# nomadoor/ComfyUI-Video-Stabilizer

Measured on AMD Instinct MI355X. Metric: stabilized frames/sec (1080p, similarity mode), higher is better.
Workload: dtype f32; 1 GPU; C2: 256-frame clip, 1920x1080, Video Stabilizer Flow (DIS) similarity + crop_and_pad, defaults (strength 0.7, smooth 0.5, 16 fps), device-resident in/out, entered at the node's input adaptation; frames_per_gpu=256, total_frames=256

## Files before the change

### comfyui-video-stabilizer_amd/csrc/vstab_api.hip

```cpp
#include "vstab_internal.h"
#include <cmath>
#include <cstdarg>

static thread_local char g_err[1024] = "";

void vstab_set_error(const char* fmt, ...)
{
    va_list ap;
    va_start(ap, fmt);
    vsnprintf(g_err, sizeof(g_err), fmt, ap);
    va_end(ap);
}

int ScratchBuf::reserve(size_t need)
{
    if (need <= bytes) return 0;
    size_t want = need + need / 4 + 256;
    if (ptr) {
        if (pinned_host) (void)hipHostFree(ptr);
        else (void)hipFree(ptr);
        ptr = nullptr;
        bytes = 0;
    }
    hipError_t e = pinned_host ? hipHostMalloc(&ptr, want, hipHostMallocDefault) : hipMalloc(&ptr, want);
    if (e != hipSuccess) {
        vstab_set_error("scratch allocation of %zu bytes failed: %s", want, hipGetErrorString(e));
        ptr = nullptr;
        return 1;
    }
    bytes = want;
    return 0;
}

void ScratchBuf::release()
{
    if (ptr) {
        if (pinned_host) (void)hipHostFree(ptr);
        else (void)hipFree(ptr);
    }
    ptr = nullptr;
    bytes = 0;
}

bool vstab_invert3x3(const double* S, double* D) { return vstab_invert3x3_hd(S, D); }

int vstab_stage_params(vstab_ctx* ctx, const void* host, size_t bytes, void** dev_out)
{
    VSTAB_HIP(hipEventSynchronize(ctx->ev_params_free));
    if (ctx->h_params.reserve(bytes)) return 1;
    if (ctx->d_params.reserve(bytes)) return 1;
    memcpy(ctx->h_params.ptr, host, bytes);
    VSTAB_HIP(hipMemcpyAsync(ctx->d_params.ptr, ctx->h_params.ptr, bytes, hipMemcpyHostToDevice, ctx->stream));
    VSTAB_HIP(hipEventRecord(ctx->ev_params_free, ctx->stream));
    *dev_out = ctx->d_params.ptr;
    return 0;
}

EventPair* vstab_timer_slot(vstab_ctx* ctx, const char* kind)
{
    auto it = ctx->timers.find(kind);
    if (it == ctx->timers.end()) {
        EventPair ep;
        if (hipEventCreate(&ep.start) != hipSuccess || hipEventCreate(&ep.stop) != hipSuccess) return nullptr;
        it = ctx->timers.emplace(kind, ep).first;
    }
    return &it->second;
}

int vstab_timer_fold(EventPair* ev)
{
    if (!ev->pending) return 0;
    float ms = 0.f;
    VSTAB_HIP(hipEventSynchronize(ev->stop));
    VSTAB_HIP(hipEventElapsedTime(&ms, ev->start, ev->stop));
    ev->total_ms += ms;
    ev->launches += 1;
    ev->pending = false;
    return 0;
}

int vstab_check_device_status(vstab_ctx* ctx, const char* who)
{
    if (!ctx || !ctx->h_status) return 0;
// ... 9 lines not shown
    return 3;
}

void vstab_tvl1_release(vstab_ctx* ctx);

extern "C" {

int vstab_abi_version(void) { return VSTAB_ABI_VERSION; }

int vstab_test_hooks(void)
{
#ifdef VSTAB_TEST_HOOKS
    return 1;
#else
    return 0;
#endif
}

const char* vstab_last_error(void) { return g_err; }

int vstab_create(vstab_ctx** out, int device)
{
    VSTAB_REQUIRE(out != nullptr, "vstab_create: out is NULL");
    int count = 0;
    VSTAB_HIP(hipGetDeviceCount(&count));
    VSTAB_REQUIRE(count > 0, "vstab_create: no HIP device visible");
    if (device < 0) VSTAB_HIP(hipGetDevice(&device));
    VSTAB_REQUIRE(device < count, "vstab_create: device %d out of range (%d visible)", device, count);
    VSTAB_HIP(hipSetDevice(device));
    vstab_ctx* ctx = new vstab_ctx();
    ctx->device = device;
    ctx->h_params.pinned_host = true;
    ctx->h_fit.pinned_host = true;
    ctx->h_xfer.pinned_host = true;
    VSTAB_HIP(hipEventCreateWithFlags(&ctx->ev_params_free, hipEventDisableTiming));
    VSTAB_HIP(hipEventRecord(ctx->ev_params_free, nullptr));
    {
        void* h = nullptr;
        VSTAB_HIP(hipHostMalloc(&h, 64, hipHostMallocMapped | hipHostMallocCoherent));
        memset(h, 0, 64);
        void* d = nullptr;
        VSTAB_HIP(hipHostGetDevicePointer(&d, h, 0));
        ctx->h_status = static_cast<volatile int*>(h);
        ctx->d_status = static_cast<int*>(d);
    }
    *out = ctx;
    return 0;
}

int vstab_destroy(vstab_ctx* ctx)
{
    if (!ctx) return 0;
    (void)hipSetDevice(ctx->device);
    (void)hipStreamSynchronize(ctx->stream);
    ctx->h_params.release();
    ctx->d_params.release();
    ctx->d_dis.release();
    vstab_tvl1_release(ctx);
    ctx->d_fit.release();
    ctx->h_fit.release();
    ctx->d_gray_tmp.release();
    ctx->d_range.release();
    ctx->d_mask_rows.release();
    ctx->d_plan.release();
    ctx->h_plan.release();
    if (ctx->h_peaks) (void)hipHostFree(ctx->h_peaks);
    if (ctx->d_peaks_count) (void)hipFree(ctx->d_peaks_count);
    if (ctx->h_counts) (void)hipHostFree(ctx->h_counts);
    if (ctx->ev_fit_done) (void)hipEventDestroy(ctx->ev_fit_done);
    if (ctx->ev_plan_done) (void)hipEventDestroy(ctx->ev_plan_done);
    if (ctx->side_stream) { (void)hipStreamSynchronize(ctx->side_stream); (void)hipStreamDestroy(ctx->side_stream); }
    if (ctx->ev_side) (void)hipEventDestroy(ctx->ev_side);
    for (auto& kv : ctx->timers) { (void)hipEventDestroy(kv.second.start); (void)hipEventDestroy(kv.second.stop); }
    (void)hipEventDestroy(ctx->ev_params_free);
    if (ctx->h_status) (void)hipHostFree(const_cast<int*>(ctx->h_status));
    if (ctx->xfer_stream) { (void)hipStreamSynchronize(ctx->xfer_stream); (void)hipStreamDestroy(ctx->xfer_stream); }
    for (auto& ev : ctx->ev_xfer) if (ev) (void)hipEventDestroy(ev);
    if (ctx->ev_xfer_sync) (void)hipEventDestroy(ctx->ev_xfer_sync);
    ctx->h_xfer.release();
    ctx->d_xfer.release();
    if (ctx->prep_stream) { (void)hipStreamSynchronize(ctx->prep_stream); (void)hipStreamDestroy(ctx->prep_stream); }
    for (auto& ev : ctx->ev_prep) if (ev) (void)hipEventDestroy(ev);
    if (ctx->ev_pyramid) (void)hipEventDestroy(ctx->ev_pyramid);
    delete ctx;
    return 0;
}

int vstab_set_stream(vstab_ctx* ctx, void* hip_stream)
{
    VSTAB_REQUIRE(ctx != nullptr, "vstab_set_stream: ctx is NULL");
    ctx->stream = reinterpret_cast<hipStream_t>(hip_stream);
    return 0;
}

int vstab_synchronize(vstab_ctx* ctx)
{
    VSTAB_REQUIRE(ctx != nullptr, "vstab_synchronize: ctx is NULL");
    VSTAB_HIP(hipStreamSynchronize(ctx->stream));
    return vstab_check_device_status(ctx, "vstab_synchronize");
}


int vstab_set_timing(vstab_ctx* ctx, int enabled)
{
    VSTAB_REQUIRE(ctx != nullptr, "vstab_set_timing: ctx is NULL");
    ctx->timing = enabled != 0;
    ctx->timing_detail = enabled == 2;
    ctx->timing_warp_only = enabled == 3;
    for (auto& kv : ctx->timers) { kv.second.pending = false; kv.second.total_ms = 0.0; kv.second.launches = 0; }
    return 0;
}

int vstab_last_kernel_ms(vstab_ctx* ctx, const char* kind, float* ms_out)
{
    VSTAB_REQUIRE(ctx != nullptr && kind != nullptr && ms_out != nullptr, "vstab_last_kernel_ms: NULL argument");
    auto it = ctx->timers.find(kind);
    VSTAB_REQUIRE(it != ctx->timers.end() && it->second.start != nullptr && (it->second.pending || it->second.launches > 0),
                  "vstab_last_kernel_ms: no timing recorded for '%s'", kind);
    VSTAB_HIP(hipEventSynchronize(it->second.stop));
    VSTAB_HIP(hipEventElapsedTime(ms_out, it->second.start, it->second.stop));
    return 0;
}

int vstab_kernel_ms_stats(vstab_ctx* ctx, const char* kind, double* total_ms, int* launches)
{
    VSTAB_REQUIRE(ctx != nullptr && kind != nullptr && total_ms != nullptr && launches != nullptr, "vstab_kernel_ms_stats: NULL argument");
    auto it = ctx->timers.find(kind);
    VSTAB_REQUIRE(it != ctx->timers.end(), "vstab_kernel_ms_stats: no timing recorded for '%s'", kind);
    if (int rc = vstab_timer_fold(&it->second)) return rc;
    *total_ms = it->second.total_ms;
    *launches = it->second.launches;
    return 0;
}

int vstab_host_math(int op, const double* a, const double* b, int n, double* out)
{
    VSTAB_REQUIRE(a != nullptr && out != nullptr && n >= 0, "vstab_host_math: bad argument");
    VSTAB_REQUIRE(op >= VSTAB_HOST_SQRT && op <= VSTAB_HOST_SIN, "vstab_host_math: unknown op %d", op);
    VSTAB_REQUIRE(op != VSTAB_HOST_ATAN2 || b != nullptr, "vstab_host_math: atan2 needs two inputs");
    for (int i = 0; i < n; i++) {
        switch (op) {
        case VSTAB_HOST_SQRT: out[i] = std::sqrt(a[i]); break;
        case VSTAB_HOST_ATAN2: out[i] = std::atan2(a[i], b[i]); break;
        case VSTAB_HOST_LOG: out[i] = std::log(a[i]); break;
        case VSTAB_HOST_EXP: out[i] = std::exp(a[i]); break;
        case VSTAB_HOST_COS: out[i] = std::cos(a[i]); break;
        default: out[i] = std::sin(a[i]); break;
        }
    }
    return 0;
}

int vstab_transitions_to_params(const float* work_mats, int count, int mode, const double* up, const double* down,
                                float* full_mats, double* params)
{
    VSTAB_REQUIRE(count >= 0 && (count == 0 || (work_mats && full_mats && params)), "vstab_transitions_to_params: bad argument");
    VSTAB_REQUIRE(mode >= VSTAB_MODE_TRANSLATION && mode <= VSTAB_MODE_PERSPECTIVE, "vstab_transitions_to_params: unknown mode %d", mode);
    VSTAB_REQUIRE((up == nullptr) == (down == nullptr), "vstab_transitions_to_params: up and down come together");
    for (int n = 0; n < count; n++) {
        const float* M = work_mats + (size_t)n * 9;
        float* F = full_mats + (size_t)n * 9;
        for (int i = 0; i < 3; i++)
            for (int j = 0; j < 3; j++) {
                if (up) {
                    const double t = up[i] * (double)M[i * 3 + j];
                    F[i * 3 + j] = (float)(t * down[j]);
// ... 85 lines not shown
```

### comfyui-video-stabilizer_amd/csrc/vstab_dis.hip

```cpp
#include "vstab_internal.h"
#include <cstdlib>
#include <cfloat>
#include <algorithm>
#include <cmath>
#include <memory>

namespace {

constexpr float DIS_EPS = 0.001f;
constexpr float DIS_INF = 1e10f;
constexpr int DIS_BORDER = 16;
constexpr int PSZ = 8;
constexpr int PSTR = 4;
constexpr int DEFAULT_FINEST = 2;
constexpr int GD_ITERS = 25;
constexpr int VAR_ITERS = 5;
constexpr int SOR_ITERS = 5;
constexpr int MAX_LEVELS = 16;

struct LevelGeom {
    int w, h, ws, hs;
};

unsigned grid_for(long long items, int block = 256)
{
    long long b = (items + block - 1) / block;
    const long long cap = 256LL * 32;
    if (b > cap) b = cap;
    if (b < 1) b = 1;
    return (unsigned)b;
}

dim3 frame_grid(long long per_frame, int frames, int block = 256)
{
    long long b = (per_frame + block - 1) / block;
    const long long cap = std::max(1LL, (256LL * 32) / std::max(frames, 1));
    if (b > cap) b = cap;
    if (b < 1) b = 1;
    return dim3((unsigned)b, (unsigned)frames);
}

#define FRAME_STRIDE(t, per_frame) \
    for (unsigned t = blockIdx.x * blockDim.x + threadIdx.x; t < (unsigned)(per_frame); t += gridDim.x * blockDim.x)

__device__ __forceinline__ int d_ceil(double v) { int i = (int)v; return i + (i < v); }
__device__ __forceinline__ int d_floor(double v) { int i = (int)v; return i - (i > v); }
__device__ __forceinline__ int f_floor(float v) { int i = (int)v; return i - (i > v); }
__device__ __forceinline__ int clampi(int v, int lo, int hi) { return v < lo ? lo : (v > hi ? hi : v); }
__device__ __forceinline__ int sat_u8_round(float v)
{
    int i = (int)__builtin_rintf(v);
    return i < 0 ? 0 : (i > 255 ? 255 : i);
}
__device__ __forceinline__ int sat_short(int v) { return v < -32768 ? -32768 : (v > 32767 ? 32767 : v); }
__device__ __forceinline__ int reflect101(int p, int len)
{
    if (len == 1) return 0;
    while (p < 0 || p >= len) {
        if (p < 0) p = -p;
        else p = 2 * len - 2 - p;
    }
    return p;
}

struct AreaAxis { int n; int si[8]; float a[8]; };

__device__ __forceinline__ void area_axis(int d, int ssize, double scale, AreaAxis& ax)
{
    const double fsx1 = d * scale, fsx2 = fsx1 + scale;
    const double cell = scale < ssize - fsx1 ? scale : ssize - fsx1;
    int sx1 = d_ceil(fsx1), sx2 = d_floor(fsx2);
    sx2 = sx2 < ssize - 1 ? sx2 : ssize - 1;
    sx1 = sx1 < sx2 ? sx1 : sx2;
    int k = 0;
    if (sx1 - fsx1 > 1e-3) { ax.si[k] = sx1 - 1; ax.a[k++] = (float)((sx1 - fsx1) / cell); }
    for (int sx = sx1; sx < sx2 && k < 7; sx++) { ax.si[k] = sx; ax.a[k++] = (float)(1.0 / cell); }
    if (fsx2 - sx2 > 1e-3 && k < 8) {
        double a = fsx2 - sx2;
        a = a < 1. ? a : 1.;
        a = a < cell ? a : cell;
        ax.si[k] = sx2; ax.a[k++] = (float)(a / cell);
    }
    ax.n = k;
}

__global__ __launch_bounds__(256) void area_u8_kernel(const uint8_t* __restrict__ src, uint8_t* __restrict__ dst, int n, int sh,
                                                      int sw, int dh, int dw, int mode, int kx, int ky, double scale_x,
                                                      double scale_y)
// ... 1167 lines not shown
        int sx, sy;
        float fx, fy;
        lin_coord(dx, scale_x, sw, sx, fx);
        if (sx < 0) { fx = 0; sx = 0; }
        if (sx >= sw - 1) { fx = 0; sx = sw - 1; }
        lin_coord(dy, scale_y, sh, sy, fy);
        const int sy0 = clampi(sy, 0, sh - 1), sy1 = clampi(sy + 1, 0, sh - 1);
        const int sx1 = sx + 1 < sw ? sx + 1 : sx;
        const float a0 = 1.f - fx, a1 = fx, b0 = 1.f - fy, b1 = fy;
        const float* S0 = sU + (p * sh + sy0) * sw;
        const float* S1 = sU + (p * sh + sy1) * sw;
        float r0 = S0[sx] * a0 + S0[sx1] * a1, r1 = S1[sx] * a0 + S1[sx1] * a1;
        out[t * 2] = (r0 * b0 + r1 * b1) * mul;
        S0 = sV + (p * sh + sy0) * sw;
        S1 = sV + (p * sh + sy1) * sw;
        r0 = S0[sx] * a0 + S0[sx1] * a1; r1 = S1[sx] * a0 + S1[sx1] * a1;
        out[t * 2 + 1] = (r0 * b0 + r1 * b1) * mul;
    }
}

int coarsest_scale(int h, int w)
{
    const int mx = w > h ? w : h, mn = w < h ? w : h;
    const int a = (int)(std::log(mx / (4.0 * PSZ)) / std::log(2.0) + 0.5);
    const int b = (int)(std::log((double)(mn / PSZ)) / std::log(2.0));
    return a < b ? a : b;
}

struct Carver {
    char* base;
    size_t off = 0;
    explicit Carver(void* p) : base(static_cast<char*>(p)) {}
    template <typename T> T* take(size_t count)
    {
        off = (off + 255) & ~size_t(255);
        T* p = base ? reinterpret_cast<T*>(base + off) : nullptr;
        off += count * sizeof(T);
        return p;
    }
};

struct AreaPlan { double scale_x, scale_y; int isx, isy, mode; };
int plan_area(int sh, int sw, int dh, int dw, AreaPlan& pl)
{
    pl.scale_x = 1. / ((double)dw / sw); pl.scale_y = 1. / ((double)dh / sh);
    pl.isx = (int)std::lrint(pl.scale_x); pl.isy = (int)std::lrint(pl.scale_y);
    const bool fast = std::fabs(pl.scale_x - pl.isx) < DBL_EPSILON && std::fabs(pl.scale_y - pl.isy) < DBL_EPSILON;
    VSTAB_REQUIRE(pl.scale_x >= 1.0 && pl.scale_y >= 1.0 && pl.scale_x < 6.0 && pl.scale_y < 6.0, "dis: area ratio %.3fx%.3f unsupported", pl.scale_x, pl.scale_y);
    pl.mode = fast ? ((pl.isx == 2 && pl.isy == 2) ? 0 : 1) : 2;
    return 0;
}

int launch_area(hipStream_t st, const uint8_t* src, uint8_t* dst, int n, int sh, int sw, int dh, int dw)
{
    AreaPlan pl;
    if (int rc = plan_area(sh, sw, dh, dw, pl)) return rc;
    const double scale_x = pl.scale_x, scale_y = pl.scale_y;
    const int isx = pl.isx, isy = pl.isy;
    int mode = pl.mode;
    if (mode == 1 && isx == 4 && isy == 4 && sw % 4 == 0 && (reinterpret_cast<uintptr_t>(src) & 3) == 0) mode = 3;
    const long long row_groups = (long long)n * ((dh + AREA_ROWS - 1) / AREA_ROWS);
    if (mode == 2 && dw <= AREA_MAX_COLS && row_groups < 0x7fffffffLL)
        hipLaunchKernelGGL(area_general_rows_kernel, dim3((unsigned)row_groups), dim3(256), 0, st, src, dst, n, sh, sw, dh, dw, scale_x, scale_y);
    else
        hipLaunchKernelGGL(area_u8_kernel, frame_grid((long long)dh * dw, n), dim3(256), 0, st, src, dst, n, sh, sw, dh, dw, mode, isx, isy, scale_x, scale_y);
    VSTAB_HIP(hipGetLastError());
    return 0;
}

}

static bool dis_scales(int h, int w, int& finest, int& coarsest)
{
    coarsest = coarsest_scale(h, w);
    if (coarsest < 0) return false;
    if (coarsest < finest) {
        const int c = (int)std::floor(std::log2((2.0f * (float)w) / (5.0f * (float)PSZ)));
        coarsest = c > 0 ? c : 0;
        finest = coarsest - 2 > 0 ? coarsest - 2 : 0;
    }
    return coarsest < MAX_LEVELS;
}

static int dis_run(vstab_ctx* ctx, const uint8_t* gray, int n, int h, int w, int FINEST, int coarsest, float* flow, float* grid_flow,
                   int sample_step)
{
    hipStream_t st = ctx->stream;
    const int P = n - 1;
    VSTAB_REQUIRE(n <= 65535, "vstab_dis_flow_batch: %d frames in one call (the frame index is a grid dimension: at most 65535)", n);
    LevelGeom G[MAX_LEVELS];
    {
        int fraction = 1, ch = 0, cw = 0;
        for (int i = 0; i <= coarsest; i++) {
            if (i == FINEST) { ch = h / fraction; cw = w / fraction; }
            else if (i > FINEST) { ch = ch / 2; cw = cw / 2; }
            if (i >= FINEST) {
                G[i].h = ch; G[i].w = cw;
                G[i].ws = 1 + (cw - PSZ) / PSTR;
                G[i].hs = 1 + (ch - PSZ) / PSTR;
                VSTAB_REQUIRE(ch >= PSZ && cw >= PSZ, "vstab_dis_flow_batch: pyramid level %d is %dx%d, smaller than a patch", i, cw, ch);
            }
            fraction *= 2;
        }
    }
    uint8_t* I[MAX_LEVELS]; uint8_t* Iext[MAX_LEVELS]; short* Ixs[MAX_LEVELS]; short* Iys[MAX_LEVELS];
    float* tensor[MAX_LEVELS]; float* Ul[MAX_LEVELS]; float* Vl[MAX_LEVELS];
    float *aux = nullptr, *aux_c = nullptr, *Sx = nullptr, *Sy = nullptr;
    VrBufs vb{};
    const LevelGeom& F = G[FINEST];
    const size_t npF = (size_t)P * F.h * F.w;
    auto layout = [&](Carver& c) {
        for (int i = FINEST; i <= coarsest; i++) {
            const size_t px = (size_t)n * G[i].h * G[i].w;
            I[i] = c.take<uint8_t>(px);
            Iext[i] = c.take<uint8_t>((size_t)n * (G[i].h + 2 * DIS_BORDER) * (G[i].w + 2 * DIS_BORDER));
            Ixs[i] = c.take<short>(px);
            Iys[i] = c.take<short>(px);
            tensor[i] = c.take<float>(5 * (size_t)n * G[i].hs * G[i].ws);
            Ul[i] = c.take<float>((size_t)P * G[i].h * G[i].w);
            Vl[i] = c.take<float>((size_t)P * G[i].h * G[i].w);
        }
        aux = c.take<float>(5 * (size_t)n * F.h * F.ws);
        aux_c = c.take<float>(5 * (size_t)n * G[coarsest].h * G[coarsest].ws);
        Sx = c.take<float>((size_t)P * F.hs * F.ws);
        Sy = c.take<float>((size_t)P * F.hs * F.ws);
        vb.avg = c.take<float>(npF); vb.Iz = c.take<float>(npF);
        vb.D0 = c.take<f4_t>(npF); vb.D1 = c.take<f4_t>(npF);
        vb.UV = c.take<f2_t>(npF); vb.dA = c.take<f2_t>(npF); vb.dB = c.take<f2_t>(npF);
    };
    {
        Carver sizer(nullptr);
        layout(sizer);
        if (ctx->d_dis.reserve(sizer.off + 256)) return 1;
    }
    Carver carver(ctx->d_dis.ptr);
    layout(carver);

    static const bool two_streams = [] { const char* e = getenv("VSTAB_DIS_PREP_STREAM"); return !(e && atoi(e) == 0); }();
    static_assert(sizeof(ctx->ev_prep) / sizeof(ctx->ev_prep[0]) >= MAX_LEVELS, "one event per pyramid level");
    hipStream_t ps = st;
    if (two_streams) {
        if (!ctx->prep_stream) {
            VSTAB_HIP(hipStreamCreateWithFlags(&ctx->prep_stream, hipStreamNonBlocking));
            VSTAB_HIP(hipEventCreateWithFlags(&ctx->ev_pyramid, hipEventDisableTiming));
            for (auto& ev : ctx->ev_prep) VSTAB_HIP(hipEventCreateWithFlags(&ev, hipEventDisableTiming));
        }
        ps = ctx->prep_stream;
    }
    auto prep_timer = std::make_unique<DetailTimer>(ctx, "dis_prep");
    bool coarsest_prepared = false;
    {
        if (launch_area(st, gray, I[FINEST], n, h, w, G[FINEST].h, G[FINEST].w)) return 1;
        static const bool tail_on = [] { const char* e = getenv("VSTAB_DIS_PYRAMID_TAIL"); return !(e && atoi(e) == 0); }();
        const int tail_levels = coarsest - FINEST;
        size_t tail_lds = 0;
        if (tail_levels >= 1) {
            const LevelGeom& a0 = G[FINEST];
            const LevelGeom& a1 = G[FINEST + 1];
            tail_lds = (((size_t)a0.h * a0.w + 15) & ~size_t(15)) + (((size_t)a1.h * a1.w + 15) & ~size_t(15)) +
                       sizeof(AreaTaps) * ((size_t)a1.w + a1.h);
        }
        if (tail_on && tail_levels >= 1 && tail_levels <= TAIL_MAX_LEVELS && tail_lds <= 150 * 1024) {
            TailArgs ta{};
#ifdef VSTAB_FUSED_TRACE
            ta.dbg = g_dis_dbg ? g_dis_dbg + 16 * 7 : nullptr;
#endif
            {
                const LevelGeom& c = G[coarsest];
                const size_t off = (tail_lds + 15) & ~size_t(15);
                const size_t need = (((size_t)4 * c.h * c.w + 15) & ~size_t(15)) + sizeof(float) * 5 * (size_t)c.h * c.ws;
                if (off + need <= 150 * 1024) {
                    ta.prep_ext = Iext[coarsest]; ta.prep_ix = Ixs[coarsest]; ta.prep_iy = Iys[coarsest]; ta.prep_tensor = tensor[coarsest];
                    ta.prep_ws = c.ws; ta.prep_hs = c.hs; ta.prep_lds_off = (int)off;
                    tail_lds = off + need;
                    coarsest_prepared = true;
                }
            }
            ta.src = I[FINEST]; ta.n = n; ta.h0 = G[FINEST].h; ta.w0 = G[FINEST].w; ta.levels = tail_levels;
            for (int i = FINEST + 1; i <= coarsest; i++) {
                AreaPlan pl;
                if (int rc = plan_area(G[i - 1].h, G[i - 1].w, G[i].h, G[i].w, pl)) return rc;
                TailLevel& tl = ta.lv[i - FINEST - 1];
                tl.dst = I[i]; tl.h = G[i].h; tl.w = G[i].w; tl.mode = pl.mode; tl.kx = pl.isx; tl.ky = pl.isy;
                if (pl.mode == 2) {
                    tl.kx = (int)std::floor(pl.scale_x) + 2; tl.ky = (int)std::floor(pl.scale_y) + 2;
                }
                tl.scale_x = pl.scale_x; tl.scale_y = pl.scale_y;
            }
            if (tail_lds > 64 * 1024)
                VSTAB_HIP(hipFuncSetAttribute(reinterpret_cast<const void*>(pyramid_tail_kernel), hipFuncAttributeMaxDynamicSharedMemorySize, (int)tail_lds));
            hipLaunchKernelGGL(pyramid_tail_kernel, dim3((unsigned)n), dim3(1024), tail_lds, st, ta);
            VSTAB_HIP(hipGetLastError());
        } else {
            for (int i = FINEST + 1; i <= coarsest; i++)
                if (launch_area(st, I[i - 1], I[i], n, G[i - 1].h, G[i - 1].w, G[i].h, G[i].w)) return 1;
        }
    }
    if (two_streams) {
        VSTAB_HIP(hipEventRecord(ctx->ev_pyramid, st));
        VSTAB_HIP(hipStreamWaitEvent(ps, ctx->ev_pyramid, 0));
    }
    for (int i = coarsest; i >= FINEST; i--) {
        const LevelGeom& g = G[i];
        const bool own = i == coarsest;
        if (own && coarsest_prepared) continue;
        hipStream_t s_i = own ? st : ps;
        float* aux_i = own ? aux_c : aux;
        hipLaunchKernelGGL(pad_replicate_kernel, frame_grid((long long)(g.h + 32) * (g.w + 32), n), dim3(256), 0, s_i, I[i], Iext[i], n, g.h, g.w);
        hipLaunchKernelGGL(sobel_kernel, frame_grid((long long)g.h * g.w, n), dim3(256), 0, s_i, I[i], Ixs[i], Iys[i], n, g.h, g.w);
        hipLaunchKernelGGL(tensor_h_kernel, frame_grid((long long)g.h * g.ws, n), dim3(256), 0, s_i, Ixs[i], Iys[i], aux_i, n, g.h, g.w, g.ws);
        hipLaunchKernelGGL(tensor_v_kernel, dim3((unsigned)((g.ws + 63) / 64), (unsigned)n, 5u), dim3(64), 0, s_i, aux_i, tensor[i], n, g.h, g.ws, g.hs);
        VSTAB_HIP(hipGetLastError());
        if (two_streams && !own) VSTAB_HIP(hipEventRecord(ctx->ev_prep[i], ps));
    }
    VSTAB_HIP(hipMemsetAsync(Ul[coarsest], 0, sizeof(float) * (size_t)P * G[coarsest].h * G[coarsest].w, st));
    VSTAB_HIP(hipMemsetAsync(Vl[coarsest], 0, sizeof(float) * (size_t)P * G[coarsest].h * G[coarsest].w, st));

    prep_timer.reset();

    bool grid_fused = false;
    const float zeta = 0.1f, epsilon = 0.001f, alpha = 20.0f, delta = 5.0f, gamma = 10.0f, omega = 1.6f;
    const float zeta2 = zeta * zeta, eps2 = epsilon * epsilon, gamma2 = gamma / 2, delta2 = delta / 2, alpha2 = alpha / 4;

    for (int i = coarsest; i >= FINEST; i--) {
        const LevelGeom& g = G[i];
        PisArgs pa{};
        pa.I = I[i]; pa.Iext = Iext[i]; pa.Ix = Ixs[i]; pa.Iy = Iys[i]; pa.tensor = tensor[i];
        pa.U = Ul[i]; pa.V = Vl[i]; pa.Sx = Sx; pa.Sy = Sy;
        pa.n = n; pa.w = g.w; pa.h = g.h; pa.ws = g.ws; pa.hs = g.hs;
        pa.stripe_sz = (int)std::ceil(g.hs / 8.0);
        pa.spin_limit = 1 << 22;
#ifdef VSTAB_TEST_HOOKS
        if (const char* e = getenv("VSTAB_DEBUG_PIS_SPIN_LIMIT")) pa.spin_limit = atoi(e);
#endif
        pa.status = ctx->d_status;
        if (two_streams && i != coarsest) VSTAB_HIP(hipStreamWaitEvent(st, ctx->ev_prep[i], 0));
        const size_t lds_bytes = (((size_t)(g.w + 32) * (g.h + 32) + 15) & ~size_t(15)) + sizeof(float) * 2 * (size_t)g.hs * g.ws + sizeof(int) * 2 * (size_t)g.hs;
        VSTAB_REQUIRE(lds_bytes <= 160 * 1024, "vstab_dis_flow_batch: level %dx%d needs %zu B of LDS (> 160 KB)", g.w, g.h, lds_bytes);
        char kind_pis[24], kind_level[24];
        snprintf(kind_pis, sizeof(kind_pis), "dis_pis4_L%d", i);
        snprintf(kind_level, sizeof(kind_level), "dis_level_L%d", i);
        auto stage_timer = std::make_unique<DetailTimer>(ctx, kind_pis);
        if (pa.stripe_sz > 4) {
            if (lds_bytes > 64 * 1024)
                VSTAB_HIP(hipFuncSetAttribute(reinterpret_cast<const void*>(pis4_kernel<2>), hipFuncAttributeMaxDynamicSharedMemorySize, (int)lds_bytes));
            hipLaunchKernelGGL(pis4_kernel<2>, dim3((unsigned)P * 2), dim3(64 * 2 * PIS_STRIPES_PER_BLOCK), lds_bytes, st, pa);
        } else {
            if (lds_bytes > 64 * 1024)
                VSTAB_HIP(hipFuncSetAttribute(reinterpret_cast<const void*>(pis4_kernel<1>), hipFuncAttributeMaxDynamicSharedMemorySize, (int)lds_bytes));
            hipLaunchKernelGGL(pis4_kernel<1>, dim3((unsigned)P * 2), dim3(64 * PIS_STRIPES_PER_BLOCK), lds_bytes, st, pa);
        }
        stage_timer.reset();
        stage_timer = std::make_unique<DetailTimer>(ctx, kind_level);
        LevelArgs la{};
#ifdef VSTAB_FUSED_TRACE
        la.dbg = g_dis_dbg ? g_dis_dbg + 16 * i : nullptr;
#endif
        la.I = I[i]; la.Sx = Sx; la.Sy = Sy; la.U = Ul[i]; la.V = Vl[i]; la.vb = vb;
        la.P = P; la.h = g.h; la.w = g.w; la.ws = g.ws; la.hs = g.hs;
        la.alpha2 = alpha2; la.delta2 = delta2; la.gamma2 = gamma2; la.zeta2 = zeta2; la.eps2 = eps2; la.omega = omega;
        if (i > FINEST) {
            const LevelGeom& d = G[i - 1];
            la.nextU = Ul[i - 1]; la.nextV = Vl[i - 1]; la.nh = d.h; la.nw = d.w; la.nhs = d.hs; la.nws = d.ws;
            la.up_sx = 1. / ((double)d.w / g.w); la.up_sy = 1. / ((double)d.h / g.h);
        }
        {
            int tx = 1, ty = 1;
            auto tile_px = [&](int tx_, int ty_, int& padded) {
                const int lw = std::min((g.w + tx_ - 1) / tx_ + 2 * SOR_HALO, g.w), lh = std::min((g.h + ty_ - 1) / ty_ + 2 * SOR_HALO, g.h);
                padded = 2 * ((lw + 3) / 2) * (lh + 2);
                return ((lw + 1) / 2) * lh;
            };
            int padded = 0;
            while (tile_px(tx, ty, padded) > SOR_NPT * FUSED_T || (size_t)padded * 16 > 160 * 1024) {
                if ((g.w + tx - 1) / tx >= (g.h + ty - 1) / ty) tx++; else ty++;
                VSTAB_REQUIRE(tx <= 64 && ty <= 64, "vstab_dis_flow_batch: cannot tile a %dx%d level", g.w, g.h);
            }
            la.tiles_x = tx; la.tiles_y = ty; la.lds_plane = (padded + 3) & ~3;
        }
        const size_t vr_lds_bytes = sizeof(float) * 4 * (size_t)la.lds_plane;
        VSTAB_REQUIRE(vr_lds_bytes <= 160 * 1024, "vstab_dis_flow_batch: SOR tile needs %zu B of LDS", vr_lds_bytes);
        static const int n_cu = [&] { int v = 256; (void)hipDeviceGetAttribute(&v, hipDeviceAttributeMultiprocessorCount, ctx->device); return v; }();
        bool split = 8 * P < 7 * n_cu;
        int forced = -1;
        if (const char* e = getenv("VSTAB_DIS_SPLIT")) { forced = atoi(e); split = forced != 0; }
        if (split && forced != 2 && la.tiles_x * la.tiles_y == 1) split = false;
        const bool fuse_grid = !split && i == FINEST && grid_flow != nullptr;
        if (fuse_grid) {
            la.grid_out = grid_flow;
            la.g_h = (h + sample_step - 1) / sample_step; la.g_w = (w + sample_step - 1) / sample_step; la.g_step = sample_step;
            la.g_sx = 1. / ((double)w / F.w); la.g_sy = 1. / ((double)h / F.h); la.g_mul = (float)(1 << FINEST);
            grid_fused = true;
        }
        if (!split) {
            if (vr_lds_bytes > 64 * 1024)
                VSTAB_HIP(hipFuncSetAttribute(reinterpret_cast<const void*>(level_kernel<LEVEL_FUSED>), hipFuncAttributeMaxDynamicSharedMemorySize, (int)vr_lds_bytes));
            la.parts = 1;
            hipLaunchKernelGGL(level_kernel<LEVEL_FUSED>, dim3((unsigned)P), dim3(FUSED_T), vr_lds_bytes, st, la);
        } else {
            const int px_parts = std::max(1, std::min(64, (g.h * g.w + FUSED_T - 1) / FUSED_T));
            la.parts = px_parts;
            hipLaunchKernelGGL(level_kernel<LEVEL_PRE>, dim3((unsigned)(P * px_parts)), dim3(FUSED_T), 0, st, la);
            hipLaunchKernelGGL(level_kernel<LEVEL_DERIV>, dim3((unsigned)(P * px_parts)), dim3(FUSED_T), 0, st, la);
            if (vr_lds_bytes > 64 * 1024)
                VSTAB_HIP(hipFuncSetAttribute(reinterpret_cast<const void*>(level_kernel<LEVEL_TILE>), hipFuncAttributeMaxDynamicSharedMemorySize, (int)vr_lds_bytes));
            la.parts = la.tiles_x * la.tiles_y;
            for (int it = 0; it < VAR_ITERS; it++) {
                la.it = it;
                hipLaunchKernelGGL(level_kernel<LEVEL_TILE>, dim3((unsigned)(P * la.parts)), dim3(FUSED_T), vr_lds_bytes, st, la);
            }
            la.parts = px_parts;
            hipLaunchKernelGGL(level_kernel<LEVEL_MERGE>, dim3((unsigned)(P * px_parts)), dim3(FUSED_T), 0, st, la);
            if (la.nextU != nullptr) {
                la.parts = std::max(1, std::min(64, (la.nhs * la.nws + FUSED_T - 1) / FUSED_T));
                hipLaunchKernelGGL(level_kernel<LEVEL_UPSAMPLE>, dim3((unsigned)(P * la.parts)), dim3(FUSED_T), 0, st, la);
            }
        }
        VSTAB_HIP(hipGetLastError());
        stage_timer.reset();
    }
    DetailTimer final_timer(ctx, "dis_final");
    const double fsx = 1. / ((double)w / F.w), fsy = 1. / ((double)h / F.h);
    const float mul = (float)(1 << FINEST);
    if (grid_flow && !grid_fused) {
        const int gh = (h + sample_step - 1) / sample_step, gw = (w + sample_step - 1) / sample_step;
        hipLaunchKernelGGL(final_sample_kernel, frame_grid((long long)gh * gw, P), dim3(256), 0, st, Ul[FINEST], Vl[FINEST], grid_flow, P,
                           F.h, F.w, gh, gw, sample_step, fsx, fsy, mul);
    }
    if (flow) {
        hipLaunchKernelGGL(final_sample_kernel, frame_grid((long long)h * w, P), dim3(256), 0, st, Ul[FINEST], Vl[FINEST], flow, P, F.h, F.w,
                           h, w, 1, fsx, fsy, mul);
    }
    VSTAB_HIP(hipGetLastError());
    return 0;
}

extern "C" int vstab_dis_flow_batch(vstab_ctx* ctx, const uint8_t* gray, int n, int h, int w, float* flow, float* grid_flow,
                                    int sample_step)
{
    VSTAB_REQUIRE(ctx != nullptr, "vstab_dis_flow_batch: ctx is NULL");
    VSTAB_REQUIRE(gray != nullptr, "vstab_dis_flow_batch: gray is NULL");
    VSTAB_REQUIRE(n >= 2, "vstab_dis_flow_batch: need at least 2 frames, got %d", n);
    VSTAB_REQUIRE(flow != nullptr || grid_flow != nullptr, "vstab_dis_flow_batch: no output requested");
    VSTAB_REQUIRE(sample_step >= 1, "vstab_dis_flow_batch: sample_step must be >= 1");
    VSTAB_REQUIRE(h > 0 && w > 0, "vstab_dis_flow_batch: non-positive size");
    int f0 = DEFAULT_FINEST, c0 = 0;
    VSTAB_REQUIRE(dis_scales(h, w, f0, c0), "vstab_dis_flow_batch: %dx%d is too small for DIS (OpenCV needs width or height >= 12)", w, h);
    int f1 = f0, c1 = 0;
    VSTAB_REQUIRE(dis_scales(h, w, f1, c1), "vstab_dis_flow_batch: scale selection failed for %dx%d", w, h);
    VSTAB_HIP(hipSetDevice(ctx->device));
    KernelTimer timer(ctx, "dis");
    const bool stateful = ctx->dis_first_pair_is_clip_start && (c1 != c0 || f1 != f0);
    if (!stateful) return dis_run(ctx, gray, n, h, w, ctx->dis_first_pair_is_clip_start ? f0 : f1, ctx->dis_first_pair_is_clip_start ? c0 : c1, flow, grid_flow, sample_step);
    if (int rc = dis_run(ctx, gray, 2, h, w, f0, c0, flow, grid_flow, sample_step)) return rc;
    if (n == 2) return 0;
    const int gh = (h + sample_step - 1) / sample_step, gw = (w + sample_step - 1) / sample_step;
    return dis_run(ctx, gray + (size_t)h * w, n - 1, h, w, f1, c1, flow ? flow + (size_t)h * w * 2 : nullptr,
                   grid_flow ? grid_flow + (size_t)gh * gw * 2 : nullptr, sample_step);
}

extern "C" int vstab_dis_set_clip_start(vstab_ctx* ctx, int first_pair_is_clip_start)
{
    VSTAB_REQUIRE(ctx != nullptr, "vstab_dis_set_clip_start: ctx is NULL");
    ctx->dis_first_pair_is_clip_start = first_pair_is_clip_start != 0;
    return 0;
}
```

### comfyui-video-stabilizer_amd/csrc/vstab_gray.hip

```cpp
#include "vstab_internal.h"
#include <algorithm>
#include <cfloat>
#include <cmath>

namespace {

__device__ __forceinline__ int gray_u8(float r, float g, float b, bool fused)
{
    const float k0 = 0.299f, k1 = 0.587f, k2 = 0.114f;
    float y;
    if (fused) y = __builtin_fmaf(b, k2, __builtin_fmaf(g, k1, r * k0));
    else y = r * k0 + g * k1 + b * k2;
    float v = y * 255.0f;
    v = v < 0.f ? 0.f : (v > 255.f ? 255.f : v);
    return (int)v;
}

__device__ __forceinline__ int sat_u8_round(float v)
{
    int i = (int)__builtin_rintf(v);
    return i < 0 ? 0 : (i > 255 ? 255 : i);
}

template <int K, bool RANGE>
__global__ __launch_bounds__(1024) void gray_area_int_kernel(const float* __restrict__ frames, uint8_t* __restrict__ out,
                                                             int n, int sh, int sw, int dh, int dw, int body,
                                                             float* __restrict__ row_max)
{
    __shared__ float s_max[16];
    __shared__ int s_nan[16];
    const int y = (int)blockIdx.x % dh, f = (int)blockIdx.x / dh;
    const float* rowbase = frames + ((size_t)f * sh + (size_t)y * K) * sw * 3;
    uint8_t* D = out + ((size_t)f * dh + y) * dw;
    float vmax = -INFINITY;
    int has_nan = 0;
    const int used = dw * K;
    constexpr int U = 4 / K;
    typedef float f3_t __attribute__((ext_vector_type(3), aligned(4)));
    for (int sx0 = threadIdx.x; sx0 < used; sx0 += U * blockDim.x) {
        f3_t px[U][K];
#pragma unroll
        for (int u = 0; u < U; u++) {
            const int sx = sx0 + u * blockDim.x;
            if (sx < used) {
#pragma unroll
                for (int j = 0; j < K; j++)
                    px[u][j] = __builtin_nontemporal_load(reinterpret_cast<const f3_t*>(rowbase + (size_t)j * sw * 3 + (size_t)sx * 3));
            }
        }
#pragma unroll
        for (int u = 0; u < U; u++) {
            const int sx = sx0 + u * blockDim.x;
            if (sx < used) {
                const bool fused = sx < body;
                int sum = 0;
#pragma unroll
                for (int j = 0; j < K; j++) {
                    const float cr = px[u][j].x, cg = px[u][j].y, cb = px[u][j].z;
                    sum += gray_u8(cr, cg, cb, fused);
                    if (RANGE) {
                        vmax = __builtin_fmaxf(vmax, __builtin_fmaxf(__builtin_fmaxf(cr, cg), cb));
                        has_nan |= ((cr != cr) | (cg != cg) | (cb != cb)) ? 1 : 0;
                    }
                }
                if (K >= 2) sum += __builtin_amdgcn_update_dpp(0, sum, 0xB1, 0xf, 0xf, false);
                if (K == 4) sum += __builtin_amdgcn_update_dpp(0, sum, 0x4E, 0xf, 0xf, false);
                if ((sx & (K - 1)) == 0) {
                    int o;
                    if (K == 1) o = sum;
                    else if (K == 2) o = (sum + 2) >> 2;
                    else o = sat_u8_round(sum * (1.f / (K * K)));
                    D[sx / K] = (uint8_t)o;
                }
            }
        }
    }
    if (RANGE) {
#pragma unroll
        for (int off = 32; off > 0; off >>= 1) {
            vmax = __builtin_fmaxf(vmax, __shfl_down(vmax, off));
            has_nan |= __shfl_down(has_nan, off);
        }
        const int nw = (blockDim.x + 63) >> 6;
// ... 102 lines not shown
    const long long total = (long long)n * dh * dw;
    const float scale = 1.f / (kx * ky);
    for (long long t = (long long)blockIdx.x * blockDim.x + threadIdx.x; t < total; t += (long long)gridDim.x * blockDim.x) {
        const int x = (int)(t % dw);
        const long long r = t / dw;
        const int y = (int)(r % dh);
        const int f = (int)(r / dh);
        const uint8_t* S = src + ((size_t)f * sh + (size_t)y * ky) * sw + (size_t)x * kx;
        int sum = 0;
        for (int j = 0; j < ky; j++)
            for (int i = 0; i < kx; i++) sum += S[(size_t)j * sw + i];
        int o;
        if (kx == 2 && ky == 2) o = (sum + 2) >> 2;
        else o = sat_u8_round(sum * scale);
        dst[t] = (uint8_t)o;
    }
}

struct AreaTabEntry { int si; float alpha; };

__global__ __launch_bounds__(256) void area_general_u8_kernel(const uint8_t* __restrict__ src, uint8_t* __restrict__ dst, int n,
                                                              int sh, int sw, int dh, int dw,
                                                              const AreaTabEntry* __restrict__ xtab, const int* __restrict__ xstart,
                                                              const AreaTabEntry* __restrict__ ytab, const int* __restrict__ ystart)
{
    const long long total = (long long)n * dh * dw;
    for (long long t = (long long)blockIdx.x * blockDim.x + threadIdx.x; t < total; t += (long long)gridDim.x * blockDim.x) {
        const int x = (int)(t % dw);
        const long long r = t / dw;
        const int y = (int)(r % dh);
        const int f = (int)(r / dh);
        const uint8_t* S = src + (size_t)f * sh * sw;
        float sum = 0.f;
        const int j0 = ystart[y], j1 = ystart[y + 1];
        const int k0 = xstart[x], k1 = xstart[x + 1];
        for (int j = j0; j < j1; j++) {
            const uint8_t* row = S + (size_t)ytab[j].si * sw;
            float buf = 0.f;
            for (int k = k0; k < k1; k++) buf += row[xtab[k].si] * xtab[k].alpha;
            const float term = ytab[j].alpha * buf;
            sum = (j == j0) ? term : sum + term;
        }
        dst[t] = (uint8_t)sat_u8_round(sum);
    }
}

int ceil_d(double v) { int i = (int)v; return i + (i < v); }
int floor_d(double v) { int i = (int)v; return i - (i > v); }

void build_area_tab(int ssize, int dsize, double scale, std::vector<AreaTabEntry>& tab, std::vector<int>& start)
{
    tab.clear();
    start.assign((size_t)dsize + 1, 0);
    for (int dx = 0; dx < dsize; dx++) {
        start[dx] = (int)tab.size();
        double fsx1 = dx * scale, fsx2 = fsx1 + scale;
        double cellWidth = scale < ssize - fsx1 ? scale : ssize - fsx1;
        int sx1 = ceil_d(fsx1), sx2 = floor_d(fsx2);
        sx2 = sx2 < ssize - 1 ? sx2 : ssize - 1;
        sx1 = sx1 < sx2 ? sx1 : sx2;
        if (sx1 - fsx1 > 1e-3) tab.push_back({sx1 - 1, (float)((sx1 - fsx1) / cellWidth)});
        for (int sx = sx1; sx < sx2; sx++) tab.push_back({sx, (float)(1.0 / cellWidth)});
        if (fsx2 - sx2 > 1e-3) {
            double a = fsx2 - sx2;
            a = a < 1. ? a : 1.;
            a = a < cellWidth ? a : cellWidth;
            tab.push_back({sx2, (float)(a / cellWidth)});
        }
    }
    start[dsize] = (int)tab.size();
}

unsigned grid_for(long long items)
{
    long long b = (items + 255) / 256;
    const long long cap = 256LL * 16;
    if (b > cap) b = cap;
    if (b < 1) b = 1;
    return (unsigned)b;
}

}

static int gray_run(vstab_ctx* ctx, const float* frames, int n, int src_h, int src_w, int work_h, int work_w, uint8_t* gray,
                    float* frame_max)
{
    VSTAB_HIP(hipSetDevice(ctx->device));
    hipStream_t st = ctx->stream;
    const int body = src_w & ~7;
    KernelTimer timer(ctx, "gray");
    float* row_max = nullptr;
    int range_rows = 0;

    auto threads_for = [](int cols) {
        int best = 256;
        long long best_cost = -1;
        for (int t = 256; t <= 1024; t += 64) {
            const long long cost = (long long)((cols + t - 1) / t) * t;
            if (best_cost < 0 || cost < best_cost || (cost == best_cost && std::abs(t - 640) < std::abs(best - 640))) { best = t; best_cost = cost; }
        }
        if (const char* e = getenv("VSTAB_GRAY_THREADS")) best = atoi(e);
        return best;
    };
#define LAUNCH_GRAY(K, ROWS, OUT)                                                                                         \
    do {                                                                                                                  \
        const int threads = threads_for(src_w / K * K);                                                                   \
        if (row_max)                                                                                                      \
            hipLaunchKernelGGL((gray_area_int_kernel<K, true>), dim3((unsigned)(n * (ROWS))), dim3(threads), 0, st, frames, OUT, n, src_h, \
                               src_w, (ROWS), src_w / K, body, row_max);                                                  \
        else                                                                                                              \
            hipLaunchKernelGGL((gray_area_int_kernel<K, false>), dim3((unsigned)(n * (ROWS))), dim3(threads), 0, st, frames, OUT, n, src_h, \
                               src_w, (ROWS), src_w / K, body, row_max);                                                  \
        VSTAB_HIP(hipGetLastError());                                                                                     \
    } while (0)

    const double scale_x = 1. / ((double)work_w / src_w), scale_y = 1. / ((double)work_h / src_h);
    const int isx = (int)std::lrint(scale_x), isy = (int)std::lrint(scale_y);
    const bool same = (work_h == src_h && work_w == src_w);
    const bool fast = !same && std::fabs(scale_x - isx) < DBL_EPSILON && std::fabs(scale_y - isy) < DBL_EPSILON;
    const bool fused = fast && isx == isy && (isx == 2 || isx == 4);
    const int K = same ? 1 : (fused ? isx : 1);
    if (frame_max) {
        const int rows = (same || !fused) ? src_h : work_h;
        if (ctx->d_range.reserve(sizeof(float) * (size_t)n * rows)) return 1;
        row_max = static_cast<float*>(ctx->d_range.ptr);
        range_rows = rows;
    }
    if (same) {
        LAUNCH_GRAY(1, work_h, gray);
    } else if (fused) {
        VSTAB_REQUIRE(work_w * K == src_w && work_h * K == src_h, "vstab_gray_downscale: %dx%d is not %d x %dx%d", src_w, src_h, K, work_w, work_h);
        if (K == 2) LAUNCH_GRAY(2, work_h, gray);
        else LAUNCH_GRAY(4, work_h, gray);
    } else {
        const size_t full = (size_t)n * src_h * src_w;
        if (ctx->d_gray_tmp.reserve(full)) return 1;
        uint8_t* tmp = static_cast<uint8_t*>(ctx->d_gray_tmp.ptr);
        LAUNCH_GRAY(1, src_h, tmp);
        const long long out_items = (long long)n * work_h * work_w;
        if (fast) {
            hipLaunchKernelGGL(area_int_u8_kernel, dim3(grid_for(out_items)), dim3(256), 0, st, tmp, gray, n, src_h, src_w, work_h, work_w, isx, isy);
            VSTAB_HIP(hipGetLastError());
        } else {
            std::vector<AreaTabEntry> xtab, ytab;
            std::vector<int> xstart, ystart;
            build_area_tab(src_w, work_w, scale_x, xtab, xstart);
            build_area_tab(src_h, work_h, scale_y, ytab, ystart);
            const size_t b_xt = xtab.size() * sizeof(AreaTabEntry), b_yt = ytab.size() * sizeof(AreaTabEntry);
            const size_t b_xs = xstart.size() * sizeof(int), b_ys = ystart.size() * sizeof(int);
            std::vector<unsigned char> blob(b_xt + b_yt + b_xs + b_ys);
            memcpy(blob.data(), xtab.data(), b_xt);
            memcpy(blob.data() + b_xt, ytab.data(), b_yt);
            memcpy(blob.data() + b_xt + b_yt, xstart.data(), b_xs);
            memcpy(blob.data() + b_xt + b_yt + b_xs, ystart.data(), b_ys);
            void* d_blob = nullptr;
            if (vstab_stage_params(ctx, blob.data(), blob.size(), &d_blob)) return 1;
            unsigned char* db = static_cast<unsigned char*>(d_blob);
            hipLaunchKernelGGL(area_general_u8_kernel, dim3(grid_for(out_items)), dim3(256), 0, st, tmp, gray, n, src_h, src_w, work_h, work_w,
                               reinterpret_cast<const AreaTabEntry*>(db), reinterpret_cast<const int*>(db + b_xt + b_yt),
                               reinterpret_cast<const AreaTabEntry*>(db + b_xt), reinterpret_cast<const int*>(db + b_xt + b_yt + b_xs));
            VSTAB_HIP(hipGetLastError());
        }
    }
#undef LAUNCH_GRAY
    if (frame_max) {
        if (ctx->h_peaks_cap < n) {
            if (ctx->h_peaks) { VSTAB_HIP(hipStreamSynchronize(st)); VSTAB_HIP(hipHostFree(ctx->h_peaks)); ctx->h_peaks = nullptr; ctx->h_peaks_cap = 0; }
            const int cap = std::max(1024, n);
            void* hp = nullptr;
            VSTAB_HIP(hipHostMalloc(&hp, sizeof(float) * (size_t)cap, hipHostMallocMapped | hipHostMallocCoherent));
            void* dp = nullptr;
            VSTAB_HIP(hipHostGetDevicePointer(&dp, hp, 0));
            ctx->h_peaks = static_cast<float*>(hp); ctx->d_peaks_mirror = static_cast<float*>(dp); ctx->h_peaks_cap = cap;
        }
        if (!ctx->d_peaks_count) {
            VSTAB_HIP(hipMalloc(reinterpret_cast<void**>(&ctx->d_peaks_count), 256));
            VSTAB_HIP(hipMemsetAsync(ctx->d_peaks_count, 0, 256, st));
        }
        ctx->peaks_target += (unsigned)n;
        ctx->peaks_frames = n;
        hipLaunchKernelGGL(frame_max_kernel, dim3((unsigned)n), dim3(256), 0, st, row_max, frame_max, range_rows, ctx->d_peaks_mirror,
                           reinterpret_cast<unsigned*>(ctx->d_status) + VSTAB_PEAKS_DONE_WORD, ctx->d_peaks_count, ctx->peaks_target);
        VSTAB_HIP(hipGetLastError());
    }
    return 0;
}

static int gray_check(const char* who, vstab_ctx* ctx, const float* frames, int n, int src_h, int src_w, int work_h, int work_w,
                      const uint8_t* gray)
{
    VSTAB_REQUIRE(ctx != nullptr, "%s: ctx is NULL", who);
    VSTAB_REQUIRE(frames && gray, "%s: NULL pointer argument", who);
    VSTAB_REQUIRE(n > 0 && src_h > 0 && src_w > 0 && work_h > 0 && work_w > 0, "%s: non-positive size", who);
    VSTAB_REQUIRE(work_h <= src_h && work_w <= src_w, "%s: working size %dx%d larger than source %dx%d", who, work_w, work_h, src_w, src_h);
    return 0;
}

extern "C" int vstab_gray_downscale(vstab_ctx* ctx, const float* frames, int n, int src_h, int src_w, int work_h,
                                    int work_w, uint8_t* gray)
{
    if (int rc = gray_check("vstab_gray_downscale", ctx, frames, n, src_h, src_w, work_h, work_w, gray)) return rc;
    return gray_run(ctx, frames, n, src_h, src_w, work_h, work_w, gray, nullptr);
}

extern "C" int vstab_gray_downscale_range(vstab_ctx* ctx, const float* frames, int n, int src_h, int src_w, int work_h,
                                          int work_w, uint8_t* gray, float* frame_max)
{
    if (int rc = gray_check("vstab_gray_downscale_range", ctx, frames, n, src_h, src_w, work_h, work_w, gray)) return rc;
    VSTAB_REQUIRE(frame_max != nullptr, "vstab_gray_downscale_range: frame_max is NULL");
    return gray_run(ctx, frames, n, src_h, src_w, work_h, work_w, gray, frame_max);
}

extern "C" int vstab_last_frame_peaks(vstab_ctx* ctx, int n, float* out)
{
    VSTAB_REQUIRE(ctx != nullptr && out != nullptr, "vstab_last_frame_peaks: NULL argument");
    VSTAB_REQUIRE(ctx->h_peaks != nullptr && n == ctx->peaks_frames, "vstab_last_frame_peaks: no range pass over %d frames is pending", n);
    volatile unsigned* done = reinterpret_cast<volatile unsigned*>(ctx->h_status) + VSTAB_PEAKS_DONE_WORD;
    const unsigned target = ctx->peaks_target;
    for (long spins = 0; (int)(*done - target) < 0; spins++) {
        if (spins > 20000000L) {
            VSTAB_HIP(hipStreamSynchronize(ctx->stream));
            VSTAB_REQUIRE((int)(*done - target) >= 0, "vstab_last_frame_peaks: the range pass finished without reporting its %d frames", n);
            break;
        }
        __builtin_ia32_pause();
    }
    __atomic_thread_fence(__ATOMIC_ACQUIRE);
    memcpy(out, ctx->h_peaks, sizeof(float) * (size_t)n);
    return 0;
}

extern "C" int vstab_frame_range(vstab_ctx* ctx, const float* frames, int n, int h, int w, float* frame_max)
{
    VSTAB_REQUIRE(ctx != nullptr, "vstab_frame_range: ctx is NULL");
    VSTAB_REQUIRE(frames && frame_max, "vstab_frame_range: NULL pointer argument");
    VSTAB_REQUIRE(n > 0 && h > 0 && w > 0, "vstab_frame_range: non-positive size");
    VSTAB_HIP(hipSetDevice(ctx->device));
    hipStream_t st = ctx->stream;
    const long long per_frame = (long long)h * w * 3;
    long long piece = (long long)w * 3;
    bool vec = false;
    for (long long cand : {(long long)w * 3, (long long)w * 3 * 2, (long long)w * 3 * 4})
        if (cand % 4 == 0 && per_frame % cand == 0 && (reinterpret_cast<uintptr_t>(frames) % 16) == 0) { piece = cand; vec = true; break; }
    const long long pieces = per_frame / piece;
    VSTAB_REQUIRE((long long)n * pieces < 0x7fffffffLL && piece < 0x7fffffffLL, "vstab_frame_range: clip too large");
    if (ctx->d_range.reserve(sizeof(float) * (size_t)n * pieces)) return 1;
    float* row_max = static_cast<float*>(ctx->d_range.ptr);
    KernelTimer timer(ctx, "range");
    if (vec) hipLaunchKernelGGL(row_max_kernel<true>, dim3((unsigned)(n * pieces)), dim3(256), 0, st, frames, row_max, (int)piece);
    else hipLaunchKernelGGL(row_max_kernel<false>, dim3((unsigned)(n * pieces)), dim3(256), 0, st, frames, row_max, (int)piece);
    hipLaunchKernelGGL(frame_max_kernel, dim3((unsigned)n), dim3(256), 0, st, row_max, frame_max, (int)pieces, (float*)nullptr, (unsigned*)nullptr, (unsigned*)nullptr, 0u);
    VSTAB_HIP(hipGetLastError());
    return 0;
}

extern "C" int vstab_apply_value_range(vstab_ctx* ctx, const float* frames, int n, int h, int w, const float* frame_max, float* out)
{
    VSTAB_REQUIRE(ctx != nullptr, "vstab_apply_value_range: ctx is NULL");
    VSTAB_REQUIRE(frames && frame_max && out, "vstab_apply_value_range: NULL pointer argument");
    VSTAB_REQUIRE(n > 0 && h > 0 && w > 0, "vstab_apply_value_range: non-positive size");
    VSTAB_HIP(hipSetDevice(ctx->device));
    const long long per_frame = (long long)h * w * 3, total = per_frame * n;
    hipLaunchKernelGGL(value_range_kernel, dim3(grid_for(total)), dim3(256), 0, ctx->stream, frames, out, frame_max, per_frame, total);
    VSTAB_HIP(hipGetLastError());
    return 0;
}
```

### comfyui-video-stabilizer_amd/distributed.py

```python

from __future__ import annotations

from typing import Any, Dict, List, Optional, Sequence, Tuple

import numpy as np

import os
import time

from . import host_math as hm
from . import flow_pipeline as _fp
from .flow_pipeline import (_ESTIMATORS, _attach_motion_meta, complete_meta, resolve_flow_backend, plan_stabilization,
                            prepare_meta)


class ShardError(RuntimeError):

    def __init__(self, where: str, failed: Sequence[Tuple[int, str]]):
        self.failed = list(failed)
        detail = "; ".join(f"rank {r}: {m}" for r, m in self.failed)
        super().__init__(f"stabilize_sharded failed {where} on {len(self.failed)} rank(s) -- {detail}")


_STATUS_HEAD = 4
# ... 187 lines not shown
    try:
        if local_frames.shape[0] >= 2:
            peaks = [] if check_value_range else None
            local_records = estimate(ctx, local_frames, working_size, transform_mode, clip_start=(rank == 0), peaks_out=peaks)
            if peaks:
                rescaled, _ = hm.apply_value_range(local_frames, peaks[0], ctx)
                if rescaled is not local_frames:
                    local_frames = rescaled
                    local_records = estimate(ctx, local_frames, working_size, transform_mode, clip_start=(rank == 0))
        else:
            if check_value_range and local_frames.shape[0] == 1:
                local_frames, _ = hm.apply_value_range(local_frames, ctx.frame_range(local_frames), ctx)
            local_records = np.zeros((0, 3), native.FIT_DTYPE)
    except Exception as exc:
        failure = exc
    t0 = _lap(stats, "estimate", t0)
    records = gather_fit_records(local_records, total_frames, group=group, device=dev, failure=failure)
    t0 = _lap(stats, "gather_fits", t0)
    own = local_frames[halo:]
    plan = meta = dst = mask = None
    counts = torch.zeros((0,), dtype=torch.int32, device=own.device)
    try:
        plan = plan_stabilization(ctx, records, size, total_frames, framing_mode, transform_mode, camera_lock, strength, smooth,
                                  keep_fov, padding_rgb, fps_effective, fps_requested, estimator=estimator)
        t0 = _lap(stats, "plan", t0)
        if plan.bypass_meta is not None:
            dst, mask = own, torch.zeros((n_local, height, width), dtype=torch.float32, device=own.device)
        elif n_local > 0:
            mats = np.ascontiguousarray(plan.final_matrices[start:end], dtype=np.float32)
            dst, mask, counts = ctx.warp_batch(own, mats, plan.output_size, interp="bilinear", border=hm.border_value(padding_rgb),
                                               want_mask=True, want_count=True)
        else:
            out_w, out_h = plan.output_size
            dst = torch.empty((0, out_h, out_w, 3), dtype=torch.float32, device=own.device)
            mask = torch.empty((0, out_h, out_w), dtype=torch.float32, device=own.device)
    except Exception as exc:
        failure = exc
    bypass = plan is not None and plan.bypass_meta is not None
    per_frame = frame_counts(total_frames, world)
    if len(counts) != per_frame[rank]:
        counts = torch.zeros((per_frame[rank],), dtype=torch.int32, device=own.device)
    fetch_counts = _start_gather_counts(counts, per_frame, group=group, on_device=dev is not None, failed=failure is not None)
    t0 = _lap(stats, "warp_launch", t0)
    late: Optional[BaseException] = None
    try:
        if failure is None and want_meta and not bypass:
            meta = prepare_meta(plan)
    except Exception as exc:
        late = exc
    t0 = _lap(stats, "meta", t0)
    all_counts, bad = fetch_counts()
    _raise_if_failed("between its two collectives", _late_failures(bad, rank, failure), failure)
    if late is not None:
        raise late
    if bypass:
        return dst, mask, _attach_motion_meta(plan.bypass_meta, fps_effective, estimator)
    if want_meta:
        meta = complete_meta(meta, plan, all_counts)
    _lap(stats, "gather_counts", t0)
    if stats is not None:
        stats["device_plan"] = {"used": False, "mismatched_frames": 0}
    return dst, mask, meta


def _stabilize_sharded_device_plan(ctx, local_frames, total_frames, start, n_local, halo, size, working_size, framing_mode,
                                   transform_mode, camera_lock, strength, smooth, keep_fov, padding_rgb, fps_effective,
                                   fps_requested, group, stats, want_meta, check_value_range, t0):
    import torch.distributed as dist

    from . import native

    torch = ctx.torch
    rank, world = dist.get_rank(group), dist.get_world_size(group)
    rec_bytes = 3 * native.FIT_DTYPE.itemsize
    per_rank = transition_counts(total_frames, world)
    rows = max(max(per_rank), 1)
    send = torch.zeros((rows + 1, rec_bytes), dtype=torch.uint8, device=ctx.device)
    pairs_local = 0
    failure: Optional[BaseException] = None
    try:
        if local_frames.shape[0] >= 2:
            def launch(frames):
                peaks_ = [] if check_value_range else None
                gray = _fp._gray(ctx, frames, working_size, peaks_)
                _, grid = ctx.dis_flow_batch(gray, sample_step=_fp.SAMPLE_STEP, want_full=False, want_grid=True, clip_start=(rank == 0))
                return ctx.sample_fit_batch_begin(grid, _fp.SAMPLE_STEP, transform_mode), peaks_

            pairs_local, peaks = launch(local_frames)
            if peaks:
                rescaled, _ = hm.apply_value_range(local_frames, peaks[0], ctx)
                if rescaled is not local_frames:
                    ctx.sample_fit_batch_end(pairs_local)
                    local_frames = rescaled
                    check_value_range = False
                    pairs_local, _ = launch(local_frames)
            ctx.fit_records_copy(send, pairs_local)
        elif check_value_range and local_frames.shape[0] == 1:
            local_frames, _ = hm.apply_value_range(local_frames, ctx.frame_range(local_frames), ctx)
        if pairs_local != per_rank[rank]:
            raise ValueError(f"rank {rank} produced {pairs_local} transitions, expected {per_rank[rank]}")
    except Exception as exc:
        failure = exc
        send[rows].copy_(torch.from_numpy(_status_row(rec_bytes, exc)))
    t0 = _lap(stats, "estimate", t0)
    flat = torch.empty((world, rows + 1, rec_bytes), dtype=torch.uint8, device=ctx.device)
    on_device = dist.get_backend(group) == "nccl"
    if on_device:
        dist.all_gather_into_tensor(flat, send, group=group)
    else:
        parts = [torch.empty((rows + 1, rec_bytes), dtype=torch.uint8) for _ in range(world)]
        dist.all_gather(parts, send.cpu(), group=group)
        flat.copy_(torch.stack(parts))
    host_t = torch.empty(flat.shape, dtype=torch.uint8, pin_memory=True)
    host_t.copy_(flat, non_blocking=True)
    gathered = torch.cuda.Event()
    gathered.record()
    own = local_frames[halo:]
    out_size = size
    dst = torch.empty((0, size[1], size[0], 3), dtype=torch.float32, device=own.device)
    mask = torch.empty((0, size[1], size[0]), dtype=torch.float32, device=own.device)
    counts = torch.zeros((0,), dtype=torch.int32, device=own.device)
    late: Optional[BaseException] = None
    if failure is None:
        try:
            ctx.flow_plan_device(flat.data_ptr(), total_frames - 1, transform_mode, size, working_size, smooth, fps_effective, strength,
                                 bool(camera_lock), seg_pairs=per_rank, seg_rows=rows + 1, warp_frames=n_local, framing=framing_mode)
            if framing_mode == "expand":
                out_size = ctx.expand_canvas(ctx.flow_plan_result(total_frames, _fp.PLAN_PARAMS[transform_mode])[3])
                if out_size is None:
                    raise native.VstabError("the device plan's expand region is not finite")
                dst = torch.empty((0, out_size[1], out_size[0], 3), dtype=torch.float32, device=own.device)
                mask = torch.empty((0, out_size[1], out_size[0]), dtype=torch.float32, device=own.device)
            if n_local > 0:
                dst, mask, counts = ctx.warp_batch_planned(own, start, out_size, border=hm.border_value(padding_rgb), want_mask=True,
                                                           want_count=True)
            t0 = _lap(stats, "warp_launch", t0)
            if pairs_local:
                ctx.sample_fit_batch_end(pairs_local)
        except Exception as exc:
            late = exc
    gathered.synchronize()
    host = host_t.numpy()
    _raise_if_failed("before the exchange of the fit records", _failed_ranks(host[:, rows]), failure)
    plan = meta = None
    verdict = {"used": True, "mismatched_frames": 0}
    if late is None:
        try:
            records = np.ascontiguousarray(np.concatenate([host[r, : per_rank[r]] for r in range(world)], axis=0)).view(native.FIT_DTYPE).reshape(-1, 3)
            t0 = _lap(stats, "gather_fits", t0)
            plan = plan_stabilization(ctx, records, size, total_frames, framing_mode, transform_mode, camera_lock, strength, smooth,
                                      keep_fov, padding_rgb, fps_effective, fps_requested, estimator="flow")
            t0 = _lap(stats, "plan", t0)
            final_dev = ctx.flow_plan_result(total_frames, _fp.PLAN_PARAMS[transform_mode])[0]
            if tuple(plan.output_size) != tuple(out_size):
                if n_local > 0:
                    dst, mask, counts = ctx.warp_batch(own, np.ascontiguousarray(plan.final_matrices[start:start + n_local], np.float32),
                                                       plan.output_size, interp="bilinear", border=hm.border_value(padding_rgb),
                                                       want_mask=True, want_count=True)
                else:
                    dst = torch.empty((0, plan.output_size[1], plan.output_size[0], 3), dtype=torch.float32, device=own.device)
                    mask = torch.empty((0, plan.output_size[1], plan.output_size[0]), dtype=torch.float32, device=own.device)
                verdict["mismatched_frames"] = n_local
            elif n_local > 0:
                sub = _fp.FlowPlan(plan.final_matrices[start:start + n_local], plan.output_size, {}, {}, {}, plan.framing_mode, size, fps_effective)
                verdict["mismatched_frames"] = _fp._rewarp_mismatched(ctx, own, sub, final_dev[start:start + n_local], dst, mask, counts,
                                                                      padding_rgb)
        except Exception as exc:
            late = exc
# ... 40 lines not shown
```

### comfyui-video-stabilizer_amd/flow_pipeline.py

```python

from __future__ import annotations

import gc
import os
from dataclasses import dataclass
from typing import Any, Dict, Optional, Tuple

import numpy as np

from . import host_math as hm
from . import mesh_warp as mesh_warp_mod
from . import native
from . import scene_cuts as scene_cuts_mod
from . import temporal_fill as temporal_fill_mod
from .comfy_compat import ProgressBar, check_interrupt
from .meta_v2 import applied_motion_meta_from_arrays, applied_motion_meta_from_stabilization_warp

SAMPLE_STEP = 8


class _gc_paused:

    def __enter__(self):
        self.was = gc.isenabled()
# ... 24 lines not shown


def _backend_fields(estimator: str) -> Dict[str, Any]:
    if estimator == "flow":
        return {"flow_backend": "DIS", "flow_fallback_reason": None}
    if estimator == "flow_phase_correlate":
        return {"flow_backend": "phase_correlate", "flow_fallback_reason": _PHASE_REASON}
    if estimator == "flow_tvl1":
        return {"flow_backend": "TVL1", "flow_fallback_reason": _TVL1_REASON}
    return {}


def _attach_motion_meta(meta: Dict[str, Any], fps: float, estimator: str = "flow") -> Dict[str, Any]:
    try:
        meta["motion_meta"] = applied_motion_meta_from_stabilization_warp(
            meta["stabilization_warp"], fps=fps, source=_META_SOURCE[estimator])
    except (KeyError, TypeError, ValueError, np.linalg.LinAlgError):
        pass
    return meta


def _replay_progress(pbar, done: int, count: int, total: int, stride: int = 10) -> int:
    for upto in range(stride, count + 1, stride):
        pbar.update_absolute(done + upto, total)
    if count % stride:
        pbar.update_absolute(done + count, total)
    return done + count


_MODE_INDEX = {"translation": 0, "similarity": 1, "perspective": 2}
_MODE_NAME = ("translation", "similarity", "perspective")


def select_transitions(fit_records, requested_mode: str):
    table = fit_records if isinstance(fit_records, np.ndarray) else native.fit_table_from_dicts(fit_records)
    pairs = table.shape[0]
    usable = (table["computed"] != 0) & (table["accepted"] != 0)
    active = _MODE_INDEX[requested_mode]
    if pairs and usable[:, active].all():
        rows = table[:, active]
        return (rows["matrix"].reshape(pairs, 3, 3).astype(np.float32), [requested_mode] * pairs, rows["confidence"].tolist(),
                rows["residual"].tolist(), requested_mode)
    chosen = np.empty(pairs, dtype=np.int64)
    p = 0
    while p < pairs:
        ok = usable[p:, active]
        run = int(ok.size if ok.all() else np.argmin(ok))
        chosen[p:p + run] = active
        p += run
        if p >= pairs:
            break
        pick = -1
        for m in range(active - 1, -1, -1):
            if usable[p, m]:
                pick = m
                break
        chosen[p] = pick
        active = pick if pick >= 0 else 0
        p += 1
    idx = chosen
    safe = np.where(idx >= 0, idx, 0)
    rows = table[np.arange(pairs), safe]
    mats = rows["matrix"].reshape(pairs, 3, 3).astype(np.float32)
    confs = rows["confidence"].astype(np.float64)
    resids = rows["residual"].astype(np.float64)
    missing = idx < 0
    if missing.any():
        mats[missing] = np.eye(3, dtype=np.float32)
        confs[missing] = 0.0
        resids[missing] = 0.0
    modes = [_MODE_NAME[m] if m >= 0 else "translation" for m in chosen.tolist()]
    return mats, modes, confs.tolist(), resids.tolist(), _MODE_NAME[active]


def _gray(ctx, device_frames, working_size, peaks_out, gray_out=None):
    if peaks_out is None:
        gray = ctx.gray_downscale(device_frames, working_size)
    else:
        gray, peaks = ctx.gray_downscale(device_frames, working_size, want_range=True)
        peaks_out.append(hm.prefetch_peaks(peaks))
    if gray_out is not None:
        gray_out.append(gray)
    return gray


def estimate_transitions(ctx, device_frames, working_size, transform_mode: str, clip_start: bool = True, peaks_out=None,
                         blocked=None, gray_out=None, grid_out=None):
    gray = _gray(ctx, device_frames, working_size, peaks_out, gray_out)
    _, grid = ctx.dis_flow_batch(gray, sample_step=SAMPLE_STEP, want_full=False, want_grid=True, clip_start=clip_start)
    if grid_out is not None:
        grid_out.append(grid)
    return ctx.sample_fit_batch(grid, SAMPLE_STEP, transform_mode, blocked=blocked)


def estimate_transitions_phase(ctx, device_frames, working_size, transform_mode: str, clip_start: bool = True, peaks_out=None,
                               gray_out=None):
    gray = _gray(ctx, device_frames, working_size, peaks_out, gray_out)
    table, _ = ctx.phase_correlate_batch(gray)
    return table


def estimate_transitions_tvl1(ctx, device_frames, working_size, transform_mode: str, clip_start: bool = True, peaks_out=None,
                              blocked=None, gray_out=None, grid_out=None):
    gray = _gray(ctx, device_frames, working_size, peaks_out, gray_out)
    _, grid, _ = ctx.tvl1_flow_batch(gray, sample_step=SAMPLE_STEP, want_full=False, want_grid=True)
    if grid_out is not None:
        grid_out.append(grid)
    return ctx.sample_fit_batch(grid, SAMPLE_STEP, transform_mode, blocked=blocked)


_ESTIMATORS = {}


CLASSIC_GFTT = dict(max_corners=400, quality=0.01, min_distance=7.0, block_size=21)
CLASSIC_LK = dict(win=31, max_level=3, max_count=50, epsilon=0.01)


def estimate_transitions_classic(ctx, device_frames, working_size, transform_mode: str, clip_start: bool = True, peaks_out=None,
                                 gray_out=None):
    gray = _gray(ctx, device_frames, working_size, peaks_out, gray_out)
    corners, counts = ctx.gftt_batch(gray[:-1], **CLASSIC_GFTT)
    pairs = ctx.lk_track_batch(gray, corners, counts, **CLASSIC_LK)
    return ctx.points_fit_batch(pairs, counts, transform_mode)


_ESTIMATORS.update({"flow": estimate_transitions, "flow_phase_correlate": estimate_transitions_phase,
                    "flow_tvl1": estimate_transitions_tvl1, "classic": estimate_transitions_classic})


def _fps_fields(context: hm.VideoContext, frame_rate) -> Tuple[float, Optional[float]]:
    cand = frame_rate
    if not isinstance(cand, (int, float)) or not np.isfinite(cand) or cand <= 0.0:
        cfps = context.fps
        cand = cfps if isinstance(cfps, (int, float)) and np.isfinite(cfps) and cfps > 0.0 else 16.0
    effective = float(max(1.0, cand))
    requested = float(frame_rate) if isinstance(frame_rate, (int, float)) and frame_rate > 0.0 else None
    return effective, requested


def _host_frames(context: hm.VideoContext) -> np.ndarray:
    if context.batch is not None:
        hm.resolve_value_range(context)
        return context.batch.detach().cpu().numpy()
    if context.batch_u8 is not None:
        arr = context.batch_u8.numpy().astype(np.float32)
        arr /= 255.0
        return arr
    return np.stack([hm._ensure_rgb(f) for f in context.frames], axis=0)


@dataclass
class FlowPlan:

    final_matrices: np.ndarray
    output_size: Tuple[int, int]
    meta_head: Dict[str, Any]
    framing_meta: Dict[str, Any]
    estimated_motion: Dict[str, Any]
    framing_mode: str
    source_size: Tuple[int, int]
    fps_effective: float
    bypass_meta: Optional[Dict[str, Any]] = None
    estimator: str = "flow"


def plan_stabilization(*args, **kwargs) -> "FlowPlan":
# ... 257 lines not shown
                                      border=hm.border_value(padding_rgb), want_mask=True, want_count=True, out=dst[a:b],
                                      out_mask=mask[a:b])
            counts[a:b].copy_(c2)
    return int(bad.size)


def _temporal_fill(ctx, device_frames, dst, mask, plan, meta, radius: int) -> None:
    if radius <= 0 or plan.framing_mode == "crop":
        return
    em = plan.estimated_motion
    meta["temporal_fill"] = temporal_fill_mod.fill_on_device(
        ctx, device_frames, dst, mask, plan.final_matrices, np.asarray(em["matrices"], dtype=np.float32), em["confidences"], radius)


MASK_MARGIN_MAX = 64
_MASK_LIMITS = {
    "classic": "the Classic estimator fits tracked corners, not grid samples: it needs a masked corner detector, which does not exist yet.",
    "flow_phase_correlate": "phase correlation yields one global transform per pair: it has no samples to drop.",
}


def check_estimation_mask_request(estimator: str, mask_margin) -> int:
    margin = int(mask_margin)
    if not 0 <= margin <= MASK_MARGIN_MAX:
        raise ValueError(f"mask_margin={margin} outside [0, {MASK_MARGIN_MAX}] (working pixels)")
    if estimator in _MASK_LIMITS:
        raise ValueError(f"estimation_mask is not supported with estimator {estimator!r}: {_MASK_LIMITS[estimator]}")
    return margin


def check_estimation_mask_shape(estimation_mask, total_frames: int, size) -> None:
    width, height = size
    shape = tuple(int(v) for v in estimation_mask.shape)
    ok = (shape == (height, width)) or (len(shape) == 3 and shape[1:] == (height, width) and shape[0] in (1, total_frames))
    if not ok:
        raise ValueError(f"estimation_mask of shape {shape} does not match the clip [{total_frames},{height},{width}]: expected "
                         f"[{total_frames},{height},{width}], [1,{height},{width}] or [{height},{width}]")


def _block_grid(ctx, estimation_mask, total_frames, working_size, margin):
    torch = ctx.torch
    mask = estimation_mask if isinstance(estimation_mask, torch.Tensor) else torch.from_numpy(np.ascontiguousarray(estimation_mask, dtype=np.float32))
    if mask.device.type == "cpu" and mask.dtype == torch.float32:
        mask = ctx.upload(mask)
    return ctx.mask_block_grid(mask, total_frames, working_size, SAMPLE_STEP, margin), 1 if mask.dim() == 2 else int(mask.shape[0])


def estimation_mask_meta(fit_records, margin: int, mask_frames: int, grid_samples: int) -> Dict[str, Any]:
    admitted = np.asarray(fit_records["total_points"][:, 0], dtype=np.int64)
    fraction = (grid_samples - admitted) / float(grid_samples)
    return {"margin": int(margin), "mask_frames": int(mask_frames), "blocked_fraction_mean": float(fraction.mean()),
            "blocked_fraction_max": float(fraction.max()), "admitted_points_min": int(admitted.min())}


def _scene_segments(ctx, scene, fit_records, gray_out, transform_mode: str, total_frames: int):
    if scene.mode == "given":
        return scene_cuts_mod.segments_from_cuts(scene.cuts, total_frames), scene_cuts_mod.meta_block(scene, scene.cuts)
    gray = gray_out[0]
    sum_abs, inside = ctx.pair_residual_batch(gray, scene_cuts_mod.scoring_transitions(fit_records, transform_mode))
    scores, overlap = scene_cuts_mod.scores_and_overlap(sum_abs, inside, int(gray.shape[1]), int(gray.shape[2]))
    cuts = scene_cuts_mod.cuts_from_pairs(scene_cuts_mod.is_cut(scores, overlap, scene.threshold))
    return scene_cuts_mod.segments_from_cuts(cuts, total_frames), scene_cuts_mod.meta_block(scene, cuts, scores, overlap)


def _mesh_offsets(ctx, mesh, plan, grid, blocked, working_size, size, segments, strength, smooth, camera_lock, fps_effective):
    width, height = size
    work = working_size if working_size is not None else size
    mw, mh = mesh.vertices
    em = plan.estimated_motion
    residual, count = ctx.mesh_residual_batch(grid, SAMPLE_STEP, work, em["work_matrices"], mw, mh, blocked=blocked)
    residual, count = residual.cpu().numpy(), count.cpu().numpy()
    max_shift = mesh.max_shift_px(width)
    offsets, _ = mesh_warp_mod.plan_offsets(
        ctx.trajectory, residual, em["confidences"], segments, float(np.clip(smooth, 0.0, 1.0)), fps_effective,
        float(np.clip(strength, 0.0, 1.0)), bool(camera_lock), (1.0 / (work[0] / float(width)), 1.0 / (work[1] / float(height))), max_shift)
    return offsets, mesh_warp_mod.meta_block(mesh, max_shift, residual, count, offsets, native.MESH_MIN_SAMPLES)


def _stabilize_with_device_plan(ctx, context, device_frames, working_size, total_frames, framing_mode, transform_mode, camera_lock,
                                strength, smooth, keep_fov, padding_rgb, fps_effective, fps_requested, pbar, progress_total,
                                keep_on_device, temporal_fill=0, blocked=None, mask_info=None):
    size = (context.width, context.height)
    peaks = [] if context.range_pending else None
    gray = _gray(ctx, device_frames, working_size, peaks)
    _, grid = ctx.dis_flow_batch(gray, sample_step=SAMPLE_STEP, want_full=False, want_grid=True)
    pairs = ctx.sample_fit_batch_begin(grid, SAMPLE_STEP, transform_mode, blocked=blocked)
    ctx.flow_plan_device(ctx.fit_records_device(), pairs, transform_mode, size, working_size, smooth, fps_effective, strength,
                         bool(camera_lock), warp_frames=total_frames, framing=framing_mode)
    out_size = size
    if framing_mode == "expand":
        out_size = ctx.expand_canvas(ctx.flow_plan_result(total_frames, PLAN_PARAMS[transform_mode])[3])
        if out_size is None:
            ctx.sample_fit_batch_end(pairs)
            return None
    dst, mask, counts = ctx.warp_batch_planned(device_frames, 0, out_size, border=hm.border_value(padding_rgb), want_mask=True,
                                               want_count=True)
    fit_records = ctx.sample_fit_batch_end(pairs)
    if peaks and hm.resolve_value_range(context, peaks[0], ctx):
        return None
    progress_done = _replay_progress(pbar, 0, total_frames - 1, progress_total)
    check_interrupt()
    plan = plan_stabilization(ctx, fit_records, size, total_frames, framing_mode, transform_mode, camera_lock, strength, smooth,
                              keep_fov, padding_rgb, fps_effective, fps_requested, estimator="flow")
    meta = prepare_meta(plan)
    final_dev = ctx.flow_plan_result(total_frames, PLAN_PARAMS[transform_mode])[0]
    if tuple(plan.output_size) != tuple(out_size):
        dst, mask, counts = ctx.warp_batch(device_frames, plan.final_matrices, plan.output_size, interp="bilinear",
                                           border=hm.border_value(padding_rgb), want_mask=True, want_count=True)
        verdict = {"used": True, "mismatched_frames": total_frames}
        mirror_ok = True
    else:
        verdict = {"used": True, "mismatched_frames": _rewarp_mismatched(ctx, device_frames, plan, final_dev, dst, mask, counts, padding_rgb)}
        mirror_ok = verdict["mismatched_frames"] == 0
    _replay_progress(pbar, progress_done, total_frames, progress_total)
    meta = complete_meta(meta, plan, _counts_to_host(counts, mirrored=mirror_ok))
    if mask_info is not None:
        meta["estimation_mask"] = estimation_mask_meta(fit_records, *mask_info)
    _temporal_fill(ctx, device_frames, dst, mask, plan, meta, temporal_fill)
    check_interrupt()
    if keep_on_device:
        return hm.StabilizationResult(dst, mask.unsqueeze(-1), meta, verdict)
    return hm.StabilizationResult(dst.cpu().numpy(), mask.cpu().numpy()[..., np.newaxis], meta, verdict)


def _stabilize_frames(
    context: hm.VideoContext,
    framing_mode: str,
    transform_mode: str,
    camera_lock: bool,
    strength: float,
    smooth: float,
    keep_fov: float,
    padding_rgb: Tuple[int, int, int],
    frame_rate: float,
    *,
    ctx: Optional[native.Context] = None,
    keep_on_device: bool = False,
    estimator: str = "flow",
    temporal_fill: int = 0,
    estimation_mask=None,
    mask_margin: int = 16,
    scene_cuts=None,
    cut_threshold=None,
    mesh_warp=None,
    mesh_max_shift=None,
) -> hm.StabilizationResult:
    scene = scene_cuts_mod.check_request(scene_cuts, cut_threshold)
    mesh = mesh_warp_mod.check_request(mesh_warp, mesh_max_shift)
    if estimator not in _META_SOURCE:
        raise ValueError(f"Unknown estimator {estimator!r}; expected 'flow' or 'classic'.")
    temporal_fill = int(temporal_fill)
    if not 0 <= temporal_fill <= temporal_fill_mod.MAX_RADIUS:
        raise ValueError(f"temporal_fill={temporal_fill} outside [0, {temporal_fill_mod.MAX_RADIUS}]")
    estimator = resolve_flow_backend(estimator)
    if estimation_mask is not None:
        mask_margin = check_estimation_mask_request(estimator, mask_margin)
    if mesh is not None:
        mesh_warp_mod.check_pipeline(estimator, framing_mode, temporal_fill)
    total_frames = len(context.frames)
    fps_effective, fps_requested = _fps_fields(context, frame_rate)
    size = (context.width, context.height)
    rgb_list = [int(c) for c in padding_rgb]

    if total_frames == 0:
        meta = {
            "frames": 0,
            "note": "Empty frame sequence; nothing to stabilise.",
            "transform_mode_requested": transform_mode,
# ... 118 lines not shown
```

### comfyui-video-stabilizer_amd/native.py

```python

from __future__ import annotations

import ctypes as C
import os
from pathlib import Path
from typing import Any, Dict, Optional

import numpy as np

_PKG_DIR = Path(__file__).resolve().parent
LIB_PATH = Path(os.environ["VSTAB_LIB"]).resolve() if os.environ.get("VSTAB_LIB") else _PKG_DIR / "lib" / "libvstab.so"

INTERP = {"bilinear": 0, "bicubic": 1}
SUBPIX = {"q5": 0, "exact": 1}
MODES = {"translation": 0, "similarity": 1, "perspective": 2}
MODE_NAMES = ("translation", "similarity", "perspective")
MESH_MAX_VERTS = 65
MESH_MIN_SAMPLES = 4

DEFAULT_SUBPIX = os.environ.get("VSTAB_SUBPIX", "q5")


class VstabError(RuntimeError):
    pass
# ... 46 lines not shown
        for mi, name in enumerate(MODE_NAMES):
            cand = entry.get(name)
            if cand is None:
                continue
            row = table[p, mi]
            row["matrix"] = np.asarray(cand["matrix"], np.float32).reshape(9)
            row["confidence"] = cand["confidence"]
            row["residual"] = cand["residual"]
            row["accepted"] = 1 if cand["accepted"] else 0
            row["computed"] = 1
            row["valid_points"] = cand.get("valid_points", 0)
            row["total_points"] = cand.get("total_points", 0)
    return table


def fit_table_to_dicts(table: np.ndarray):
    out = []
    for p in range(table.shape[0]):
        entry = {}
        for mi, name in enumerate(MODE_NAMES):
            r = table[p, mi]
            if not r["computed"]:
                continue
            entry[name] = {
                "matrix": np.array(r["matrix"], dtype=np.float32).reshape(3, 3),
                "confidence": float(r["confidence"]),
                "residual": float(r["residual"]),
                "accepted": bool(r["accepted"]),
                "valid_points": int(r["valid_points"]),
                "total_points": int(r["total_points"]),
            }
        out.append(entry)
    return out


_SIGNATURES = {
    "vstab_abi_version": (C.c_int, []),
    "vstab_last_pad_counts": (C.c_int, [C.c_void_p, C.c_int, C.c_void_p]),
    "vstab_flow_plan_zero_counts": (C.c_int, [C.c_void_p, C.c_void_p, C.c_int]),
    "vstab_last_frame_peaks": (C.c_int, [C.c_void_p, C.c_int, C.c_void_p]),
    "vstab_test_hooks": (C.c_int, []),
    "vstab_last_error": (C.c_char_p, []),
    "vstab_create": (C.c_int, [C.POINTER(C.c_void_p), C.c_int]),
    "vstab_destroy": (C.c_int, [C.c_void_p]),
    "vstab_set_stream": (C.c_int, [C.c_void_p, C.c_void_p]),
    "vstab_synchronize": (C.c_int, [C.c_void_p]),
    "vstab_set_timing": (C.c_int, [C.c_void_p, C.c_int]),
    "vstab_last_kernel_ms": (C.c_int, [C.c_void_p, C.c_char_p, C.POINTER(C.c_float)]),
    "vstab_kernel_ms_stats": (C.c_int, [C.c_void_p, C.c_char_p, C.POINTER(C.c_double), C.POINTER(C.c_int)]),
    "vstab_upload": (C.c_int, [C.c_void_p, C.c_void_p, C.c_void_p, C.c_size_t]),
    "vstab_download": (C.c_int, [C.c_void_p, C.c_void_p, C.c_void_p, C.c_size_t]),
    "vstab_upload_f32_coded": (C.c_int, [C.c_void_p, C.c_void_p, C.c_void_p, C.c_size_t, C.POINTER(C.c_size_t)]),
    "vstab_upload_u8_as_f32": (C.c_int, [C.c_void_p, C.c_void_p, C.c_void_p, C.c_size_t]),
    "vstab_download_mask_levels": (C.c_int, [C.c_void_p, C.c_void_p, C.c_void_p, C.c_size_t, C.c_int, C.POINTER(C.c_int)]),
    "vstab_download_mask_coded": (C.c_int, [C.c_void_p, C.c_void_p, C.c_void_p, C.c_size_t, C.POINTER(C.c_int)]),
    "vstab_warp_batch": (
        C.c_int,
        [C.c_void_p, C.c_void_p, C.c_int, C.c_int, C.c_int, C.c_void_p, C.c_int, C.c_int, C.c_int, C.c_void_p,
         C.c_int, C.c_void_p, C.c_void_p, C.c_void_p],
    ),
    "vstab_warp_blur_batch": (
        C.c_int,
        [C.c_void_p, C.c_void_p, C.c_int, C.c_int, C.c_int, C.c_void_p, C.c_void_p, C.c_int, C.c_int, C.c_int,
         C.c_int, C.c_void_p, C.c_int, C.c_void_p, C.c_void_p],
    ),
    "vstab_warp_blur_clip_batch": (
        C.c_int,
        [C.c_void_p, C.c_void_p, C.c_int, C.c_int, C.c_int, C.c_void_p, C.c_int, C.c_int, C.c_void_p, C.c_int, C.c_int,
         C.c_int, C.c_int, C.c_void_p, C.c_int, C.c_void_p, C.c_void_p],
    ),
    "vstab_blur_sample_matrices": (
        C.c_int, [C.c_void_p, C.c_int, C.c_int, C.c_int, C.c_void_p, C.c_int, C.c_void_p]),
    "vstab_common_coverage": (
        C.c_int, [C.c_void_p, C.c_void_p, C.c_int, C.c_int, C.c_int, C.c_int, C.c_int, C.c_void_p]),
    "vstab_gray_downscale": (
        C.c_int, [C.c_void_p, C.c_void_p, C.c_int, C.c_int, C.c_int, C.c_int, C.c_int, C.c_void_p]),
    "vstab_gray_downscale_range": (
        C.c_int, [C.c_void_p, C.c_void_p, C.c_int, C.c_int, C.c_int, C.c_int, C.c_int, C.c_void_p, C.c_void_p]),
    "vstab_frame_range": (C.c_int, [C.c_void_p, C.c_void_p, C.c_int, C.c_int, C.c_int, C.c_void_p]),
    "vstab_apply_value_range": (C.c_int, [C.c_void_p, C.c_void_p, C.c_int, C.c_int, C.c_int, C.c_void_p, C.c_void_p]),
    "vstab_dis_flow_batch": (
        C.c_int, [C.c_void_p, C.c_void_p, C.c_int, C.c_int, C.c_int, C.c_void_p, C.c_void_p, C.c_int]),
    "vstab_dis_set_clip_start": (C.c_int, [C.c_void_p, C.c_int]),
    "vstab_sample_fit_batch": (
        C.c_int, [C.c_void_p, C.c_void_p, C.c_int, C.c_int, C.c_int, C.c_int, C.c_int, C.c_void_p]),
    "vstab_sample_fit_batch_begin": (C.c_int, [C.c_void_p, C.c_void_p, C.c_int, C.c_int, C.c_int, C.c_int, C.c_int]),
    "vstab_mask_block_grid": (
        C.c_int, [C.c_void_p, C.c_void_p, C.c_int, C.c_int, C.c_int, C.c_int, C.c_int, C.c_int, C.c_int, C.c_int, C.c_void_p]),
    "vstab_sample_fit_batch_masked": (
        C.c_int, [C.c_void_p, C.c_void_p, C.c_int, C.c_int, C.c_int, C.c_int, C.c_int, C.c_void_p, C.c_void_p]),
    "vstab_sample_fit_batch_begin_masked": (
        C.c_int, [C.c_void_p, C.c_void_p, C.c_int, C.c_int, C.c_int, C.c_int, C.c_int, C.c_void_p]),
    "vstab_pair_residual_batch": (
        C.c_int, [C.c_void_p, C.c_void_p, C.c_int, C.c_int, C.c_int, C.c_void_p, C.c_void_p, C.c_void_p]),
    "vstab_mesh_residual_batch": (
        C.c_int, [C.c_void_p, C.c_void_p, C.c_int, C.c_int, C.c_int, C.c_int, C.c_int, C.c_int, C.c_void_p, C.c_void_p, C.c_int,
                  C.c_int, C.c_void_p, C.c_void_p]),
    "vstab_mesh_warp_batch": (
        C.c_int, [C.c_void_p, C.c_void_p, C.c_int, C.c_int, C.c_int, C.c_void_p, C.c_int, C.c_int, C.c_void_p, C.c_int,
                  C.c_void_p, C.c_int, C.c_int, C.c_void_p, C.c_void_p, C.c_void_p]),
    "vstab_fit_records_device": (C.c_void_p, [C.c_void_p]),
    "vstab_sample_fit_batch_end": (C.c_int, [C.c_void_p, C.c_int, C.c_void_p]),
    "vstab_flow_plan_device": (
        C.c_int, [C.c_void_p, C.c_void_p, C.c_int, C.c_int, C.c_void_p, C.c_void_p, C.c_double, C.c_double, C.c_double, C.c_int,
                  C.c_int, C.c_int, C.c_int, C.c_void_p, C.c_int, C.c_int]),
    "vstab_fit_records_copy": (C.c_int, [C.c_void_p, C.c_void_p, C.c_int]),
    "vstab_flow_plan_result": (C.c_int, [C.c_void_p, C.c_int, C.c_void_p, C.c_void_p, C.c_void_p, C.c_void_p]),
    "vstab_warp_batch_planned": (
        C.c_int, [C.c_void_p, C.c_void_p, C.c_int, C.c_int, C.c_int, C.c_int, C.c_int, C.c_int, C.c_int, C.c_void_p, C.c_int,
                  C.c_void_p, C.c_void_p, C.c_void_p]),
    "vstab_temporal_fill_batch": (
        C.c_int, [C.c_void_p, C.c_void_p, C.c_int, C.c_int, C.c_int, C.c_int, C.c_int, C.c_void_p, C.c_void_p, C.c_int, C.c_int,
                  C.c_int, C.c_int, C.c_int, C.c_void_p, C.c_void_p, C.c_void_p, C.c_void_p, C.c_void_p]),
    "vstab_gftt_batch": (
        C.c_int, [C.c_void_p, C.c_void_p, C.c_int, C.c_int, C.c_int, C.c_int, C.c_double, C.c_double, C.c_int, C.c_void_p,
                  C.c_void_p]),
    "vstab_lk_levels": (C.c_int, [C.c_int, C.c_int, C.c_int, C.c_int]),
    "vstab_lk_track_batch": (
        C.c_int, [C.c_void_p, C.c_void_p, C.c_int, C.c_int, C.c_int, C.c_void_p, C.c_void_p, C.c_int, C.c_int, C.c_int,
                  C.c_int, C.c_double, C.c_void_p, C.c_void_p, C.c_void_p]),
    "vstab_points_fit_batch": (
        C.c_int, [C.c_void_p, C.c_void_p, C.c_void_p, C.c_int, C.c_int, C.c_int, C.c_void_p]),
    "vstab_phase_correlate_batch": (
        C.c_int, [C.c_void_p, C.c_void_p, C.c_int, C.c_int, C.c_int, C.c_void_p, C.c_void_p]),
    "vstab_tvl1_default_params": (None, [C.c_void_p]),
    "vstab_tvl1_flow_batch": (
        C.c_int, [C.c_void_p, C.c_void_p, C.c_int, C.c_int, C.c_int, C.c_void_p, C.c_void_p, C.c_void_p, C.c_int, C.c_void_p]),
    "vstab_host_math": (C.c_int, [C.c_int, C.c_void_p, C.c_void_p, C.c_int, C.c_void_p]),
    "vstab_transitions_to_params": (C.c_int, [C.c_void_p, C.c_int, C.c_int, C.c_void_p, C.c_void_p, C.c_void_p, C.c_void_p]),
    "vstab_params_to_matrices": (C.c_int, [C.c_void_p, C.c_int, C.c_int, C.c_void_p]),
    "vstab_bounding_boxes": (C.c_int, [C.c_void_p, C.c_int, C.c_double, C.c_double, C.c_void_p, C.c_void_p]),
    "vstab_crop_analysis": (
        C.c_int, [C.c_void_p, C.c_void_p, C.c_int, C.c_int, C.c_int, C.c_int, C.c_int, C.c_void_p, C.c_void_p]),
    "vstab_trajectory": (
        C.c_int,
        [C.c_void_p, C.c_void_p, C.c_int, C.c_int, C.c_double, C.c_double, C.c_double, C.c_int, C.c_void_p,
         C.c_void_p],
    ),
}

EXPORTED_SYMBOLS = tuple(_SIGNATURES)

_lib = None


def load_library():
    global _lib
    if _lib is None:
        if not LIB_PATH.exists():
            raise VstabError(
                f"{LIB_PATH} is missing: build it with `python -c 'import __graft_entry__ as g; g.build()'` "
                "(hipcc --offload-arch=gfx950). This package has no CPU fallback."
            )
        import torch

        lib = C.CDLL(str(LIB_PATH))
        for name, (res, args) in _SIGNATURES.items():
            fn = getattr(lib, name)
            fn.restype = res
            fn.argtypes = args
        if lib.vstab_abi_version() != 1:
            raise VstabError(f"libvstab ABI version {lib.vstab_abi_version()} != 1")
        _lib = lib
    return _lib


# ... 243 lines not shown
        self.use_torch_stream()
        _check(
            self.lib.vstab_warp_blur_clip_batch(
                self.handle, _dev_ptr(src), n, sh, sw, m.ctypes.data, total, int(clip_first), ts.ctypes.data, int(samples),
                out_h, out_w, INTERP[interp], b.ctypes.data, SUBPIX[subpix or DEFAULT_SUBPIX], _dev_ptr(dst),
                _dev_ptr(mask) if mask is not None else None,
            ),
            "vstab_warp_blur_clip_batch",
        )
        return dst, mask

    def gray_downscale(self, frames, work_size, want_range=False):
        torch = self.torch
        src = self._as_device_frames(frames)
        n, sh, sw, ch = src.shape
        if ch != 3:
            raise VstabError(f"gray_downscale expects 3-channel frames, got {ch}")
        ww, wh = (sw, sh) if work_size is None else (int(work_size[0]), int(work_size[1]))
        gray = torch.empty((n, wh, ww), dtype=torch.uint8, device=self.device)
        self.use_torch_stream()
        if want_range:
            peaks = torch.empty((n,), dtype=torch.float32, device=self.device)
            _check(self.lib.vstab_gray_downscale_range(self.handle, _dev_ptr(src), n, sh, sw, wh, ww, _dev_ptr(gray), _dev_ptr(peaks)),
                   "vstab_gray_downscale_range")
            peaks._vstab_fetch = lambda n=n: self.last_frame_peaks(n)
            return gray, peaks
        _check(self.lib.vstab_gray_downscale(self.handle, _dev_ptr(src), n, sh, sw, wh, ww, _dev_ptr(gray)),
               "vstab_gray_downscale")
        return gray

    def last_pad_counts(self, n: int) -> np.ndarray:
        out = np.empty((int(n),), np.uint32)
        _check(self.lib.vstab_last_pad_counts(self.handle, int(n), out.ctypes.data), "vstab_last_pad_counts")
        return out.astype(np.int64)

    def last_frame_peaks(self, n: int) -> np.ndarray:
        out = np.empty((int(n),), np.float32)
        _check(self.lib.vstab_last_frame_peaks(self.handle, int(n), out.ctypes.data), "vstab_last_frame_peaks")
        return out

    def frame_range(self, frames):
        torch = self.torch
        src = self._as_device_frames(frames)
        n, sh, sw, ch = src.shape
        peaks = torch.empty((n,), dtype=torch.float32, device=self.device)
        self.use_torch_stream()
        _check(self.lib.vstab_frame_range(self.handle, _dev_ptr(src), n, sh, sw * ch // 3, _dev_ptr(peaks)), "vstab_frame_range")
        return peaks

    def apply_value_range(self, frames, peaks):
        torch = self.torch
        src = self._as_device_frames(frames)
        n, sh, sw, ch = src.shape
        out = torch.empty_like(src)
        peaks = peaks.to(device=self.device, dtype=torch.float32).contiguous()
        self.use_torch_stream()
        _check(self.lib.vstab_apply_value_range(self.handle, _dev_ptr(src), n, sh, sw * ch // 3, _dev_ptr(peaks), _dev_ptr(out)),
               "vstab_apply_value_range")
        return out

    def dis_flow_batch(self, gray, sample_step=8, want_full=False, want_grid=True, clip_start=True):
        torch = self.torch
        _check(self.lib.vstab_dis_set_clip_start(self.handle, 1 if clip_start else 0), "vstab_dis_set_clip_start")
        if gray.device != self.device:
            gray = gray.to(self.device)
        gray = gray.contiguous()
        n, h, w = gray.shape
        pairs = n - 1
        if pairs < 1:
            raise VstabError("dis_flow_batch needs at least two frames")
        gh, gw = (h + sample_step - 1) // sample_step, (w + sample_step - 1) // sample_step
        flow = torch.empty((pairs, h, w, 2), dtype=torch.float32, device=self.device) if want_full else None
        grid = torch.empty((pairs, gh, gw, 2), dtype=torch.float32, device=self.device) if want_grid else None
        self.use_torch_stream()
        _check(
            self.lib.vstab_dis_flow_batch(
                self.handle, _dev_ptr(gray), n, h, w, _dev_ptr(flow) if flow is not None else None,
                _dev_ptr(grid) if grid is not None else None, int(sample_step),
            ),
            "vstab_dis_flow_batch",
        )
        return flow, grid

    def tvl1_flow_batch(self, gray, params=None, sample_step=8, want_full=False, want_grid=True, want_iterations=False):
        torch = self.torch
        if gray.device != self.device:
            gray = gray.to(self.device)
        gray = gray.contiguous()
        if gray.dtype != torch.uint8 or gray.dim() != 3:
            raise ValueError("tvl1_flow_batch expects a uint8 [N,h,w] tensor")
        n, h, w = gray.shape
        if n < 2:
            raise ValueError("tvl1_flow_batch needs at least two frames")
        if params is None:
            prm = tvl1_params()
        elif isinstance(params, Tvl1Params):
            prm = params
        else:
            prm = tvl1_params(**params)
        pairs = n - 1
        gh, gw = (h + sample_step - 1) // sample_step, (w + sample_step - 1) // sample_step
        flow = torch.empty((pairs, h, w, 2), dtype=torch.float32, device=self.device) if want_full else None
        grid = torch.empty((pairs, gh, gw, 2), dtype=torch.float32, device=self.device) if want_grid else None
        iters = (torch.empty((pairs, max(prm.nscales, 1), max(prm.warps, 1)), dtype=torch.int32, device=self.device)
                 if want_iterations else None)
        self.use_torch_stream()
        _check(
            self.lib.vstab_tvl1_flow_batch(
                self.handle, _dev_ptr(gray), n, h, w, C.byref(prm), _dev_ptr(flow) if flow is not None else None,
                _dev_ptr(grid) if grid is not None else None, int(sample_step), _dev_ptr(iters) if iters is not None else None,
            ),
            "vstab_tvl1_flow_batch",
        )
        return flow, grid, iters

    def mask_block_grid(self, mask, n_frames, working_size, step, margin):
        torch = self.torch
        if not isinstance(mask, torch.Tensor):
            mask = torch.from_numpy(np.ascontiguousarray(mask, dtype=np.float32))
        if mask.dim() == 2:
            mask = mask.unsqueeze(0)
        if mask.dim() != 3 or mask.shape[0] not in (1, int(n_frames)):
            raise ValueError(f"mask_block_grid: mask {tuple(mask.shape)} is not [{int(n_frames)},H,W], [1,H,W] or [H,W]")
        if not 0 <= int(margin) <= 64:
            raise ValueError(f"mask_block_grid: margin {margin} outside [0, 64]")
        mask = mask.to(device=self.device, dtype=torch.float32).contiguous()
        n_masks, sh, sw = (int(v) for v in mask.shape)
        ww, wh = (sw, sh) if working_size is None else (int(working_size[0]), int(working_size[1]))
        gh, gw = (wh + step - 1) // step, (ww + step - 1) // step
        blocked = torch.empty((int(n_frames), gh, gw), dtype=torch.uint8, device=self.device)
        self.use_torch_stream()
        _check(self.lib.vstab_mask_block_grid(self.handle, _dev_ptr(mask), n_masks, int(n_frames), sh, sw, wh, ww, int(step),
                                              int(margin), _dev_ptr(blocked)), "vstab_mask_block_grid")
        return blocked

    def pair_residual_batch(self, gray, transitions):
        torch = self.torch
        if gray.dtype != torch.uint8 or gray.dim() != 3:
            raise ValueError("pair_residual_batch expects a uint8 [N,h,w] tensor")
        gray = gray.to(self.device).contiguous()
        n, h, w = (int(v) for v in gray.shape)
        if n < 2:
            raise ValueError("pair_residual_batch needs at least two frames")
        m = np.ascontiguousarray(transitions, dtype=np.float32)
        if m.size != (n - 1) * 9:
            raise ValueError(f"pair_residual_batch: transitions {m.shape} are not [{n - 1},3,3] for {n} frames")
        sums = torch.empty((n - 1,), dtype=torch.int64, device=self.device)
        inside = torch.empty((n - 1,), dtype=torch.int32, device=self.device)
        self.use_torch_stream()
        _check(self.lib.vstab_pair_residual_batch(self.handle, _dev_ptr(gray), n, h, w, m.ctypes.data, _dev_ptr(sums),
                                                  _dev_ptr(inside)), "vstab_pair_residual_batch")
        return sums.cpu().numpy(), inside.cpu().numpy().astype(np.int64)

    @staticmethod
    def _check_mesh(who, mw, mh):
        if not (2 <= int(mw) <= MESH_MAX_VERTS and 2 <= int(mh) <= MESH_MAX_VERTS):
            raise ValueError(f"{who}: {mw}x{mh} vertices outside 2..{MESH_MAX_VERTS} per axis")
        return int(mw), int(mh)

    def mesh_residual_batch(self, grid_flow, step, work_size, transitions, mw, mh, blocked=None):
        torch = self.torch
        mw, mh = self._check_mesh("mesh_residual_batch", mw, mh)
        if grid_flow.dtype != torch.float32 or grid_flow.dim() != 4 or grid_flow.shape[3] != 2:
            raise ValueError("mesh_residual_batch expects a float32 [P,gh,gw,2] tensor")
        grid_flow, blocked, pairs, gh, gw = self._fit_inputs(grid_flow, blocked)
        ww, wh, step = int(work_size[0]), int(work_size[1]), int(step)
# ... 312 lines not shown
```

### include/vstab.h

```cpp
#ifndef VSTAB_H
#define VSTAB_H

#include <stddef.h>
#include <stdint.h>

#ifdef __cplusplus
extern "C" {
#endif

#define VSTAB_ABI_VERSION 1

typedef struct vstab_ctx vstab_ctx;

enum vstab_interp { VSTAB_INTERP_BILINEAR = 0, VSTAB_INTERP_BICUBIC = 1 };
enum vstab_subpix { VSTAB_SUBPIX_Q5 = 0, VSTAB_SUBPIX_EXACT = 1 };
enum vstab_mode { VSTAB_MODE_TRANSLATION = 0, VSTAB_MODE_SIMILARITY = 1, VSTAB_MODE_PERSPECTIVE = 2 };

int vstab_abi_version(void);
const char* vstab_last_error(void);
int vstab_test_hooks(void);
int vstab_create(vstab_ctx** out, int device);
int vstab_destroy(vstab_ctx* ctx);
int vstab_set_stream(vstab_ctx* ctx, void* hip_stream);
int vstab_synchronize(vstab_ctx* ctx);
int vstab_set_timing(vstab_ctx* ctx, int enabled);
int vstab_last_kernel_ms(vstab_ctx* ctx, const char* kind, float* ms_out);
int vstab_kernel_ms_stats(vstab_ctx* ctx, const char* kind, double* total_ms, int* launches);

int vstab_upload(vstab_ctx* ctx, const void* host_src, void* dev_dst, size_t bytes);
int vstab_download(vstab_ctx* ctx, const void* dev_src, void* host_dst, size_t bytes);
int vstab_upload_f32_coded(vstab_ctx* ctx, const float* host_src, float* dev_dst, size_t count, size_t* coded_chunks);
int vstab_upload_u8_as_f32(vstab_ctx* ctx, const unsigned char* host_src, float* dev_dst, size_t count);
int vstab_download_mask_coded(vstab_ctx* ctx, const float* dev_src, float* host_dst, size_t count, int* coded);
int vstab_download_mask_levels(vstab_ctx* ctx, const float* dev_src, float* host_dst, size_t count, int levels, int* coded);

int vstab_warp_batch(vstab_ctx* ctx, const float* src, int n, int src_h, int src_w,
                     const float* matrices, int out_h, int out_w, int interp,
                     const float* border_rgb, int subpix, float* dst, float* mask,
                     uint32_t* pad_count);

int vstab_warp_blur_batch(vstab_ctx* ctx, const float* src, int n, int src_h, int src_w,
                          const double* matrices, const double* ts, int samples, int out_h,
                          int out_w, int interp, const float* border_rgb, int subpix,
                          float* dst, float* mask);

int vstab_warp_blur_clip_batch(vstab_ctx* ctx, const float* src, int n, int src_h, int src_w,
                               const double* clip_matrices, int clip_total, int clip_first,
                               const double* ts, int samples, int out_h, int out_w, int interp,
                               const float* border_rgb, int subpix, float* dst, float* mask);

int vstab_blur_sample_matrices(const double* matrices, int total, int first, int count,
                               const double* ts, int samples, float* out);

int vstab_gray_downscale(vstab_ctx* ctx, const float* frames, int n, int src_h, int src_w,
                         int work_h, int work_w, uint8_t* gray);

int vstab_gray_downscale_range(vstab_ctx* ctx, const float* frames, int n, int src_h, int src_w,
                               int work_h, int work_w, uint8_t* gray, float* frame_max);
int vstab_last_frame_peaks(vstab_ctx* ctx, int n, float* out);
int vstab_frame_range(vstab_ctx* ctx, const float* frames, int n, int h, int w, float* frame_max);
int vstab_apply_value_range(vstab_ctx* ctx, const float* frames, int n, int h, int w,
                            const float* frame_max, float* out);

int vstab_dis_flow_batch(vstab_ctx* ctx, const uint8_t* gray, int n, int h, int w,
                         float* flow, float* grid_flow, int sample_step);

int vstab_dis_set_clip_start(vstab_ctx* ctx, int first_pair_is_clip_start);

typedef struct vstab_fit_record {
    float matrix[9];
    double confidence;
    double residual;
    int32_t accepted;
    int32_t computed;
    int32_t valid_points;
    int32_t total_points;
} vstab_fit_record;
int vstab_sample_fit_batch(vstab_ctx* ctx, const float* grid_flow, int pairs, int gh, int gw,
                           int step, int requested_mode, vstab_fit_record* results);
int vstab_sample_fit_batch_begin(vstab_ctx* ctx, const float* grid_flow, int pairs, int gh, int gw,
                                 int step, int requested_mode);
const vstab_fit_record* vstab_fit_records_device(vstab_ctx* ctx);
int vstab_sample_fit_batch_end(vstab_ctx* ctx, int pairs, vstab_fit_record* results);

int vstab_mask_block_grid(vstab_ctx* ctx, const float* mask, int n_masks, int n_frames, int src_h, int src_w,
                          int work_h, int work_w, int step, int margin, uint8_t* blocked);
int vstab_sample_fit_batch_masked(vstab_ctx* ctx, const float* grid_flow, int pairs, int gh, int gw,
                                  int step, int requested_mode, const uint8_t* blocked, vstab_fit_record* results);
int vstab_sample_fit_batch_begin_masked(vstab_ctx* ctx, const float* grid_flow, int pairs, int gh, int gw,
                                        int step, int requested_mode, const uint8_t* blocked);

int vstab_pair_residual_batch(vstab_ctx* ctx, const uint8_t* gray, int n, int h, int w, const float* transitions,
                              uint64_t* sum_abs, uint32_t* inside);

int vstab_crop_analysis(vstab_ctx* ctx, const float* matrices, int n, int src_h, int src_w,
                        int out_h, int out_w, int32_t* bbox, uint8_t* common);

int vstab_common_coverage(vstab_ctx* ctx, const float* matrices, int n, int src_h, int src_w,
                          int out_h, int out_w, uint8_t* common);

int vstab_gftt_batch(vstab_ctx* ctx, const uint8_t* gray, int n, int h, int w, int max_corners,
                     double quality, double min_distance, int block_size, float* corners, int* counts);
int vstab_lk_levels(int h, int w, int win, int max_level);
int vstab_lk_track_batch(vstab_ctx* ctx, const uint8_t* gray, int n, int h, int w, const float* points,
                         const int* counts, int max_points, int win, int max_level, int max_count,
                         double epsilon, float* point_pairs, float* next_points, uint8_t* status);
int vstab_points_fit_batch(vstab_ctx* ctx, const float* point_pairs, const int* counts, int pairs,
                           int max_points, int requested_mode, vstab_fit_record* results);

int vstab_phase_correlate_batch(vstab_ctx* ctx, const uint8_t* gray, int n, int h, int w,
                                vstab_fit_record* results, double* shifts);

typedef struct vstab_tvl1_params {
    double tau, lambda, theta, epsilon, scale_step, gamma;
    int nscales, warps, inner_iterations, outer_iterations, median_filtering, use_initial_flow;
    int chunk_pairs, poll_interval;
} vstab_tvl1_params;
void vstab_tvl1_default_params(vstab_tvl1_params* params);
int vstab_tvl1_flow_batch(vstab_ctx* ctx, const uint8_t* gray, int n, int h, int w, const vstab_tvl1_params* params,
                          float* flow, float* grid_flow, int sample_step, int32_t* iterations);

int vstab_trajectory(vstab_ctx* ctx, const double* deltas, int n, int p, double smooth,
                     double fps, double strength, int camera_lock, double* path,
                     double* target);

int vstab_flow_plan_zero_counts(vstab_ctx* ctx, uint32_t* pad_count, int n);
int vstab_flow_plan_device(vstab_ctx* ctx, const vstab_fit_record* d_records, int pairs, int requested_mode,
                           const double* up, const double* down, double smooth, double fps, double strength,
                           int camera_lock, int width, int height, int segments, const int* seg_pairs, int seg_rows, int framing);
int vstab_fit_records_copy(vstab_ctx* ctx, void* dst_dev, int pairs);
int vstab_flow_plan_result(vstab_ctx* ctx, int frames, float* final32, double* path, double* target, double* region);
int vstab_warp_batch_planned(vstab_ctx* ctx, const float* src, int first, int n, int src_h, int src_w, int out_h,
                             int out_w, int interp, const float* border_rgb, int subpix, float* dst, float* mask,
                             uint32_t* pad_count);
int vstab_last_pad_counts(vstab_ctx* ctx, int n, uint32_t* out);

int vstab_temporal_fill_batch(vstab_ctx* ctx, const float* src, int clip_frames, int src_h, int src_w, int first, int n,
                              const float* matrices, const int32_t* cand_frame, int K, int out_h, int out_w, int interp,
                              int subpix, float* dst, float* mask, int8_t* filled_from, uint32_t* fill_count,
                              uint32_t* pad_count);

#define VSTAB_MESH_MIN_SAMPLES 4
int vstab_mesh_residual_batch(vstab_ctx* ctx, const float* grid_flow, int pairs, int gh, int gw, int step, int work_h,
                              int work_w, const float* transitions, const uint8_t* blocked, int mw, int mh,
                              float* residual, int32_t* count);
int vstab_mesh_warp_batch(vstab_ctx* ctx, const float* src, int n, int src_h, int src_w, const float* matrices,
                          int out_h, int out_w, const float* border_rgb, int subpix, const float* offsets, int mw, int mh,
                          float* dst, float* mask, uint32_t* pad_count);

enum { VSTAB_HOST_SQRT = 0, VSTAB_HOST_ATAN2 = 1, VSTAB_HOST_LOG = 2, VSTAB_HOST_EXP = 3, VSTAB_HOST_COS = 4, VSTAB_HOST_SIN = 5 };
// ... 13 lines not shown
```

Measured before the change: 32380 frames/s.

## Fuse grayscale downscale with DIS flow and pipeline front/tail frame chunks

Adds a combined gray+DIS entry point that plans DIS buffers once and can split the frame batch at a boundary, so the grayscale conversion, pyramid prep and per-level DIS work for early frames can run while later frames are still being converted. DIS setup is refactored into plan, per-level prep and per-level solve helpers that take frame and pair offsets. The Python pipeline now calls this single native entry instead of two separate calls. This adds complexity and extra streams/events, and overlap only happens when the boundary setting enables splitting.

```diff
diff --git a/comfyui-video-stabilizer_amd/csrc/vstab_api.hip b/comfyui-video-stabilizer_amd/csrc/vstab_api.hip
--- a/comfyui-video-stabilizer_amd/csrc/vstab_api.hip
+++ b/comfyui-video-stabilizer_amd/csrc/vstab_api.hip
@@ -1,4 +1,5 @@
 #include "vstab_internal.h"
+#include "vstab_front.h"
 #include <cmath>
 #include <cstdarg>
 
@@ -174,6 +175,7 @@
     if (ctx->prep_stream) { (void)hipStreamSynchronize(ctx->prep_stream); (void)hipStreamDestroy(ctx->prep_stream); }
     for (auto& ev : ctx->ev_prep) if (ev) (void)hipEventDestroy(ev);
     if (ctx->ev_pyramid) (void)hipEventDestroy(ctx->ev_pyramid);
+    vstab_front_release(ctx);
     delete ctx;
     return 0;
 }
diff --git a/comfyui-video-stabilizer_amd/csrc/vstab_dis.hip b/comfyui-video-stabilizer_amd/csrc/vstab_dis.hip
--- a/comfyui-video-stabilizer_amd/csrc/vstab_dis.hip
+++ b/comfyui-video-stabilizer_amd/csrc/vstab_dis.hip
@@ -1,9 +1,11 @@
 #include "vstab_internal.h"
+#include "vstab_front.h"
 #include <cstdlib>
 #include <cfloat>
 #include <algorithm>
 #include <cmath>
 #include <memory>
+#include <mutex>
 
 namespace {
 
@@ -1337,13 +1339,32 @@
     return coarsest < MAX_LEVELS;
 }
 
-static int dis_run(vstab_ctx* ctx, const uint8_t* gray, int n, int h, int w, int FINEST, int coarsest, float* flow, float* grid_flow,
-                   int sample_step)
-{
-    hipStream_t st = ctx->stream;
-    const int P = n - 1;
+static bool dis_fused_form(vstab_ctx* ctx, int P)
+{
+    static const int n_cu = [&] { int v = 256; (void)hipDeviceGetAttribute(&v, hipDeviceAttributeMultiprocessorCount, ctx->device); return v; }();
+    return 8 * P >= 7 * n_cu;
+}
+
+constexpr int FRONT_TAIL_DIVISOR = 4;
+
+struct DisPlan {
+    int n = 0, P = 0, h = 0, w = 0, FINEST = 0, coarsest = 0;
+    LevelGeom G[MAX_LEVELS];
+    uint8_t* I[MAX_LEVELS]; uint8_t* Iext[MAX_LEVELS]; short* Ixs[MAX_LEVELS]; short* Iys[MAX_LEVELS];
+    float* tensor[MAX_LEVELS]; float* Ul[MAX_LEVELS]; float* Vl[MAX_LEVELS];
+    float *aux = nullptr, *aux_c = nullptr, *aux_in = nullptr, *Sx = nullptr, *Sy = nullptr;
+    VrBufs vb{};
+    bool two_streams = false;
+    hipStream_t ps = nullptr;
+    bool grid_fused = false;
+};
+
+static int dis_plan(vstab_ctx* ctx, int n, int h, int w, int FINEST, int coarsest, DisPlan& D)
+{
+    D.n = n; D.P = n - 1; D.h = h; D.w = w; D.FINEST = FINEST; D.coarsest = coarsest;
+    const int P = D.P;
     VSTAB_REQUIRE(n <= 65535, "vstab_dis_flow_batch: %d frames in one call (the frame index is a grid dimension: at most 65535)", n);
-    LevelGeom G[MAX_LEVELS];
+    LevelGeom* G = D.G;
     {
         int fraction = 1, ch = 0, cw = 0;
         for (int i = 0; i <= coarsest; i++) {
@@ -1358,30 +1379,27 @@
             fraction *= 2;
         }
     }
-    uint8_t* I[MAX_LEVELS]; uint8_t* Iext[MAX_LEVELS]; short* Ixs[MAX_LEVELS]; short* Iys[MAX_LEVELS];
-    float* tensor[MAX_LEVELS]; float* Ul[MAX_LEVELS]; float* Vl[MAX_LEVELS];
-    float *aux = nullptr, *aux_c = nullptr, *Sx = nullptr, *Sy = nullptr;
-    VrBufs vb{};
     const LevelGeom& F = G[FINEST];
     const size_t npF = (size_t)P * F.h * F.w;
     auto layout = [&](Carver& c) {
         for (int i = FINEST; i <= coarsest; i++) {
             const size_t px = (size_t)n * G[i].h * G[i].w;
-            I[i] = c.take<uint8_t>(px);
-            Iext[i] = c.take<uint8_t>((size_t)n * (G[i].h + 2 * DIS_BORDER) * (G[i].w + 2 * DIS_BORDER));
-            Ixs[i] = c.take<short>(px);
-            Iys[i] = c.take<short>(px);
-            tensor[i] = c.take<float>(5 * (size_t)n * G[i].hs * G[i].ws);
-            Ul[i] = c.take<float>((size_t)P * G[i].h * G[i].w);
-            Vl[i] = c.take<float>((size_t)P * G[i].h * G[i].w);
-        }
-        aux = c.take<float>(5 * (size_t)n * F.h * F.ws);
-        aux_c = c.take<float>(5 * (size_t)n * G[coarsest].h * G[coarsest].ws);
-        Sx = c.take<float>((size_t)P * F.hs * F.ws);
-        Sy = c.take<float>((size_t)P * F.hs * F.ws);
-        vb.avg = c.take<float>(npF); vb.Iz = c.take<float>(npF);
-        vb.D0 = c.take<f4_t>(npF); vb.D1 = c.take<f4_t>(npF);
-        vb.UV = c.take<f2_t>(npF); vb.dA = c.take<f2_t>(npF); vb.dB = c.take<f2_t>(npF);
+            D.I[i] = c.take<uint8_t>(px);
+            D.Iext[i] = c.take<uint8_t>((size_t)n * (G[i].h + 2 * DIS_BORDER) * (G[i].w + 2 * DIS_BORDER));
+            D.Ixs[i] = c.take<short>(px);
+            D.Iys[i] = c.take<short>(px);
+            D.tensor[i] = c.take<float>(5 * (size_t)n * G[i].hs * G[i].ws);
+            D.Ul[i] = c.take<float>((size_t)P * G[i].h * G[i].w);
+            D.Vl[i] = c.take<float>((size_t)P * G[i].h * G[i].w);
+        }
+        D.aux = c.take<float>(5 * (size_t)n * F.h * F.ws);
+        D.aux_c = c.take<float>(5 * (size_t)n * G[coarsest].h * G[coarsest].ws);
+        D.Sx = c.take<float>((size_t)P * F.hs * F.ws);
+        D.Sy = c.take<float>((size_t)P * F.hs * F.ws);
+        D.vb.avg = c.take<float>(npF); D.vb.Iz = c.take<float>(npF);
+        D.vb.D0 = c.take<f4_t>(npF); D.vb.D1 = c.take<f4_t>(npF);
+        D.vb.UV = c.take<f2_t>(npF); D.vb.dA = c.take<f2_t>(npF); D.vb.dB = c.take<f2_t>(npF);
+        if (coarsest > FINEST) D.aux_in = c.take<float>(5 * (size_t)n * G[FINEST + 1].h * G[FINEST + 1].ws);
     };
     {
         Carver sizer(nullptr);
@@ -1393,19 +1411,166 @@
 
     static const bool two_streams = [] { const char* e = getenv("VSTAB_DIS_PREP_STREAM"); return !(e && atoi(e) == 0); }();
     static_assert(sizeof(ctx->ev_prep) / sizeof(ctx->ev_prep[0]) >= MAX_LEVELS, "one event per pyramid level");
-    hipStream_t ps = st;
+    D.two_streams = two_streams;
+    D.ps = ctx->stream;
     if (two_streams) {
         if (!ctx->prep_stream) {
             VSTAB_HIP(hipStreamCreateWithFlags(&ctx->prep_stream, hipStreamNonBlocking));
             VSTAB_HIP(hipEventCreateWithFlags(&ctx->ev_pyramid, hipEventDisableTiming));
             for (auto& ev : ctx->ev_prep) VSTAB_HIP(hipEventCreateWithFlags(&ev, hipEventDisableTiming));
         }
-        ps = ctx->prep_stream;
-    }
+        D.ps = ctx->prep_stream;
+    }
+    return 0;
+}
+
+static int dis_prep_level(const DisPlan& D, int i, int f0, int cnt, hipStream_t s, float* aux)
+{
+    const LevelGeom& g = D.G[i];
+    const int n = D.n;
+    const size_t px = (size_t)f0 * g.h * g.w;
+    const uint8_t* I = D.I[i] + px;
+    short* Ix = D.Ixs[i] + px;
+    short* Iy = D.Iys[i] + px;
+    float* aux_f = aux + (size_t)f0 * g.h * g.ws;
+    hipLaunchKernelGGL(pad_replicate_kernel, frame_grid((long long)(g.h + 32) * (g.w + 32), cnt), dim3(256), 0, s, I,
+                       D.Iext[i] + (size_t)f0 * (g.h + 2 * DIS_BORDER) * (g.w + 2 * DIS_BORDER), cnt, g.h, g.w);
+    hipLaunchKernelGGL(sobel_kernel, frame_grid((long long)g.h * g.w, cnt), dim3(256), 0, s, I, Ix, Iy, cnt, g.h, g.w);
+    hipLaunchKernelGGL(tensor_h_kernel, frame_grid((long long)g.h * g.ws, cnt), dim3(256), 0, s, Ix, Iy, aux_f, n, g.h, g.w, g.ws);
+    hipLaunchKernelGGL(tensor_v_kernel, dim3((unsigned)((g.ws + 63) / 64), (unsigned)cnt, 5u), dim3(64), 0, s, aux_f,
+                       D.tensor[i] + (size_t)f0 * g.hs * g.ws, n, g.h, g.ws, g.hs);
+    VSTAB_HIP(hipGetLastError());
+    return 0;
+}
+
+static int dis_level(vstab_ctx* ctx, DisPlan& D, int i, int p0, int pc, hipStream_t st, float* grid_flow, int sample_step)
+{
+    if (pc <= 0) return 0;
+    const int n = D.n, P = D.P, h = D.h, w = D.w, FINEST = D.FINEST, coarsest = D.coarsest;
+    const LevelGeom* G = D.G;
+    const LevelGeom& F = G[FINEST];
+    const LevelGeom& g = G[i];
+    const float zeta = 0.1f, epsilon = 0.001f, alpha = 20.0f, delta = 5.0f, gamma = 10.0f, omega = 1.6f;
+    const float zeta2 = zeta * zeta, eps2 = epsilon * epsilon, gamma2 = gamma / 2, delta2 = delta / 2, alpha2 = alpha / 4;
+    const size_t px0 = (size_t)p0 * g.h * g.w;
+    float* Sx = D.Sx + (size_t)p0 * F.hs * F.ws;
+    float* Sy = D.Sy + (size_t)p0 * F.hs * F.ws;
+    VrBufs vb = D.vb;
+    {
+        const size_t s0 = (size_t)p0 * F.h * F.w;
+        vb.avg += s0; vb.Iz += s0; vb.D0 += s0; vb.D1 += s0; vb.UV += s0; vb.dA += s0; vb.dB += s0;
+    }
+    PisArgs pa{};
+    pa.I = D.I[i] + px0; pa.Iext = D.Iext[i] + (size_t)p0 * (g.h + 2 * DIS_BORDER) * (g.w + 2 * DIS_BORDER);
+    pa.Ix = D.Ixs[i] + px0; pa.Iy = D.Iys[i] + px0; pa.tensor = D.tensor[i] + (size_t)p0 * g.hs * g.ws;
+    pa.U = D.Ul[i] + px0; pa.V = D.Vl[i] + px0; pa.Sx = Sx; pa.Sy = Sy;
+    pa.n = n; pa.w = g.w; pa.h = g.h; pa.ws = g.ws; pa.hs = g.hs;
+    pa.stripe_sz = (int)std::ceil(g.hs / 8.0);
+    pa.spin_limit = 1 << 22;
+#ifdef VSTAB_TEST_HOOKS
+    if (const char* e = getenv("VSTAB_DEBUG_PIS_SPIN_LIMIT")) pa.spin_limit = atoi(e);
+#endif
+    pa.status = ctx->d_status;
+    const size_t lds_bytes = (((size_t)(g.w + 32) * (g.h + 32) + 15) & ~size_t(15)) + sizeof(float) * 2 * (size_t)g.hs * g.ws + sizeof(int) * 2 * (size_t)g.hs;
+    VSTAB_REQUIRE(lds_bytes <= 160 * 1024, "vstab_dis_flow_batch: level %dx%d needs %zu B of LDS (> 160 KB)", g.w, g.h, lds_bytes);
+    char kind_pis[24], kind_level[24];
+    snprintf(kind_pis, sizeof(kind_pis), "dis_pis4_L%d", i);
+    snprintf(kind_level, sizeof(kind_level), "dis_level_L%d", i);
+    auto stage_timer = std::make_unique<DetailTimer>(ctx, kind_pis);
+    if (pa.stripe_sz > 4) {
+        if (lds_bytes > 64 * 1024)
+            VSTAB_HIP(hipFuncSetAttribute(reinterpret_cast<const void*>(pis4_kernel<2>), hipFuncAttributeMaxDynamicSharedMemorySize, (int)lds_bytes));
+        hipLaunchKernelGGL(pis4_kernel<2>, dim3((unsigned)pc * 2), dim3(64 * 2 * PIS_STRIPES_PER_BLOCK), lds_bytes, st, pa);
+    } else {
+        if (lds_bytes > 64 * 1024)
+            VSTAB_HIP(hipFuncSetAttribute(reinterpret_cast<const void*>(pis4_kernel<1>), hipFuncAttributeMaxDynamicSharedMemorySize, (int)lds_bytes));
+        hipLaunchKernelGGL(pis4_kernel<1>, dim3((unsigned)pc * 2), dim3(64 * PIS_STRIPES_PER_BLOCK), lds_bytes, st, pa);
+    }
+    stage_timer.reset();
+    stage_timer = std::make_unique<DetailTimer>(ctx, kind_level);
+    LevelArgs la{};
+#ifdef VSTAB_FUSED_TRACE
+    la.dbg = g_dis_dbg ? g_dis_dbg + 16 * i : nullptr;
+#endif
+    la.I = D.I[i] + px0; la.Sx = Sx; la.Sy = Sy; la.U = D.Ul[i] + px0; la.V = D.Vl[i] + px0; la.vb = vb;
+    la.P = pc; la.h = g.h; la.w = g.w; la.ws = g.ws; la.hs = g.hs;
+    la.alpha2 = alpha2; la.delta2 = delta2; la.gamma2 = gamma2; la.zeta2 = zeta2; la.eps2 = eps2; la.omega = omega;
+    if (i > FINEST) {
+        const LevelGeom& d = G[i - 1];
+        la.nextU = D.Ul[i - 1] + (size_t)p0 * d.h * d.w; la.nextV = D.Vl[i - 1] + (size_t)p0 * d.h * d.w;
+        la.nh = d.h; la.nw = d.w; la.nhs = d.hs; la.nws = d.ws;
+        la.up_sx = 1. / ((double)d.w / g.w); la.up_sy = 1. / ((double)d.h / g.h);
+    }
+    {
+        int tx = 1, ty = 1;
+        auto tile_px = [&](int tx_, int ty_, int& padded) {
+            const int lw = std::min((g.w + tx_ - 1) / tx_ + 2 * SOR_HALO, g.w), lh = std::min((g.h + ty_ - 1) / ty_ + 2 * SOR_HALO, g.h);
+            padded = 2 * ((lw + 3) / 2) * (lh + 2);
+            return ((lw + 1) / 2) * lh;
+        };
+        int padded = 0;
+        while (tile_px(tx, ty, padded) > SOR_NPT * FUSED_T || (size_t)padded * 16 > 160 * 1024) {
+            if ((g.w + tx - 1) / tx >= (g.h + ty - 1) / ty) tx++; else ty++;
+            VSTAB_REQUIRE(tx <= 64 && ty <= 64, "vstab_dis_flow_batch: cannot tile a %dx%d level", g.w, g.h);
+        }
+        la.tiles_x = tx; la.tiles_y = ty; la.lds_plane = (padded + 3) & ~3;
+    }
+    const size_t vr_lds_bytes = sizeof(float) * 4 * (size_t)la.lds_plane;
+    VSTAB_REQUIRE(vr_lds_bytes <= 160 * 1024, "vstab_dis_flow_batch: SOR tile needs %zu B of LDS", vr_lds_bytes);
+    bool split = !dis_fused_form(ctx, P);
+    int forced = -1;
+    if (const char* e = getenv("VSTAB_DIS_SPLIT")) { forced = atoi(e); split = forced != 0; }
+    if (split && forced != 2 && la.tiles_x * la.tiles_y == 1) split = false;
+    const bool fuse_grid = !split && i == FINEST && grid_flow != nullptr;
+    if (fuse_grid) {
+        la.grid_out = grid_flow;
+        la.g_h = (h + sample_step - 1) / sample_step; la.g_w = (w + sample_step - 1) / sample_step; la.g_step = sample_step;
+        la.g_sx = 1. / ((double)w / F.w); la.g_sy = 1. / ((double)h / F.h); la.g_mul = (float)(1 << FINEST);
+        D.grid_fused = true;
+    }
+    if (!split) {
+        if (vr_lds_bytes > 64 * 1024)
+            VSTAB_HIP(hipFuncSetAttribute(reinterpret_cast<const void*>(level_kernel<LEVEL_FUSED>), hipFuncAttributeMaxDynamicSharedMemorySize, (int)vr_lds_bytes));
+        la.parts = 1;
+        hipLaunchKernelGGL(level_kernel<LEVEL_FUSED>, dim3((unsigned)pc), dim3(FUSED_T), vr_lds_bytes, st, la);
+    } else {
+        const int px_parts = std::max(1, std::min(64, (g.h * g.w + FUSED_T - 1) / FUSED_T));
+        la.parts = px_parts;
+        hipLaunchKernelGGL(level_kernel<LEVEL_PRE>, dim3((unsigned)(pc * px_parts)), dim3(FUSED_T), 0, st, la);
+        hipLaunchKernelGGL(level_kernel<LEVEL_DERIV>, dim3((unsigned)(pc * px_parts)), dim3(FUSED_T), 0, st, la);
+        if (vr_lds_bytes > 64 * 1024)
+            VSTAB_HIP(hipFuncSetAttribute(reinterpret_cast<const void*>(level_kernel<LEVEL_TILE>), hipFuncAttributeMaxDynamicSharedMemorySize, (int)vr_lds_bytes));
+        la.parts = la.tiles_x * la.tiles_y;
+        for (int it = 0; it < VAR_ITERS; it++) {
+            la.it = it;
+            hipLaunchKernelGGL(level_kernel<LEVEL_TILE>, dim3((unsigned)(pc * la.parts)), dim3(FUSED_T), vr_lds_bytes, st, la);
+        }
+        la.parts = px_parts;
+        hipLaunchKernelGGL(level_kernel<LEVEL_MERGE>, dim3((unsigned)(pc * px_parts)), dim3(FUSED_T), 0, st, la);
+        if (la.nextU != nullptr) {
+            la.parts = std::max(1, std::min(64, (la.nhs * la.nws + FUSED_T - 1) / FUSED_T));
+            hipLaunchKernelGGL(level_kernel<LEVEL_UPSAMPLE>, dim3((unsigned)(pc * la.parts)), dim3(FUSED_T), 0, st, la);
+        }
+    }
+    VSTAB_HIP(hipGetLastError());
+    stage_timer.reset();
+    (void)coarsest;
+    return 0;
+}
+
+static int dis_front(vstab_ctx* ctx, DisPlan& D, const uint8_t* gray, int f0, int f1, int p0, int p1, hipStream_t st, bool inline_prep,
+                     bool finest_prep, hipEvent_t other_pyramid, hipEvent_t pyramid_done)
+{
+    const int n = D.n, h = D.h, w = D.w, FINEST = D.FINEST, coarsest = D.coarsest;
+    const int cnt = f1 - f0, pc = p1 - p0;
+    const LevelGeom* G = D.G;
+    const bool two_streams = D.two_streams;
+    hipStream_t ps = inline_prep ? st : D.ps;
     auto prep_timer = std::make_unique<DetailTimer>(ctx, "dis_prep");
     bool coarsest_prepared = false;
-    {
-        if (launch_area(st, gray, I[FINEST], n, h, w, G[FINEST].h, G[FINEST].w)) return 1;
+    auto at = [&](uint8_t* base, int i, int f) { return base + (size_t)f * G[i].h * G[i].w; };
+    if (cnt > 0) {
+        if (launch_area(st, gray + (size_t)f0 * h * w, at(D.I[FINEST], FINEST, f0), cnt, h, w, G[FINEST].h, G[FINEST].w)) return 1;
         static const bool tail_on = [] { const char* e = getenv("VSTAB_DIS_PYRAMID_TAIL"); return !(e && atoi(e) == 0); }();
         const int tail_levels = coarsest - FINEST;
         size_t tail_lds = 0;
@@ -1425,18 +1590,20 @@
                 const size_t off = (tail_lds + 15) & ~size_t(15);
                 const size_t need = (((size_t)4 * c.h * c.w + 15) & ~size_t(15)) + sizeof(float) * 5 * (size_t)c.h * c.ws;
                 if (off + need <= 150 * 1024) {
-                    ta.prep_ext = Iext[coarsest]; ta.prep_ix = Ixs[coarsest]; ta.prep_iy = Iys[coarsest]; ta.prep_tensor = tensor[coarsest];
+                    ta.prep_ext = D.Iext[coarsest] + (size_t)f0 * (c.h + 2 * DIS_BORDER) * (c.w + 2 * DIS_BORDER);
+                    ta.prep_ix = D.Ixs[coarsest] + (size_t)f0 * c.h * c.w; ta.prep_iy = D.Iys[coarsest] + (size_t)f0 * c.h * c.w;
+                    ta.prep_tensor = D.tensor[coarsest] + (size_t)f0 * c.hs * c.ws;
                     ta.prep_ws = c.ws; ta.prep_hs = c.hs; ta.prep_lds_off = (int)off;
                     tail_lds = off + need;
                     coarsest_prepared = true;
                 }
             }
-            ta.src = I[FINEST]; ta.n = n; ta.h0 = G[FINEST].h; ta.w0 = G[FINEST].w; ta.levels = tail_levels;
+            ta.src = at(D.I[FINEST], FINEST, f0); ta.n = n; ta.h0 = G[FINEST].h; ta.w0 = G[FINEST].w; ta.levels = tail_levels;
             for (int i = FINEST + 1; i <= coarsest; i++) {
                 AreaPlan pl;
                 if (int rc = plan_area(G[i - 1].h, G[i - 1].w, G[i].h, G[i].w, pl)) return rc;
                 TailLevel& tl = ta.lv[i - FINEST - 1];
-                tl.dst = I[i]; tl.h = G[i].h; tl.w = G[i].w; tl.mode = pl.mode; tl.kx = pl.isx; tl.ky = pl.isy;
+                tl.dst = at(D.I[i], i, f0); tl.h = G[i].h; tl.w = G[i].w; tl.mode = pl.mode; tl.kx = pl.isx; tl.ky = pl.isy;
                 if (pl.mode == 2) {
                     tl.kx = (int)std::floor(pl.scale_x) + 2; tl.ky = (int)std::floor(pl.scale_y) + 2;
                 }
@@ -1444,150 +1611,99 @@
             }
             if (tail_lds > 64 * 1024)
                 VSTAB_HIP(hipFuncSetAttribute(reinterpret_cast<const void*>(pyramid_tail_kernel), hipFuncAttributeMaxDynamicSharedMemorySize, (int)tail_lds));
-            hipLaunchKernelGGL(pyramid_tail_kernel, dim3((unsigned)n), dim3(1024), tail_lds, st, ta);
+            hipLaunchKernelGGL(pyramid_tail_kernel, dim3((unsigned)cnt), dim3(1024), tail_lds, st, ta);
             VSTAB_HIP(hipGetLastError());
         } else {
             for (int i = FINEST + 1; i <= coarsest; i++)
-                if (launch_area(st, I[i - 1], I[i], n, G[i - 1].h, G[i - 1].w, G[i].h, G[i].w)) return 1;
-        }
-    }
-    if (two_streams) {
+                if (launch_area(st, at(D.I[i - 1], i - 1, f0), at(D.I[i], i, f0), cnt, G[i - 1].h, G[i - 1].w, G[i].h, G[i].w)) return 1;
+        }
+    }
+    if (two_streams && !inline_prep) {
         VSTAB_HIP(hipEventRecord(ctx->ev_pyramid, st));
         VSTAB_HIP(hipStreamWaitEvent(ps, ctx->ev_pyramid, 0));
     }
     for (int i = coarsest; i >= FINEST; i--) {
-        const LevelGeom& g = G[i];
+        if (i == FINEST && !finest_prep) continue;
         const bool own = i == coarsest;
         if (own && coarsest_prepared) continue;
-        hipStream_t s_i = own ? st : ps;
-        float* aux_i = own ? aux_c : aux;
-        hipLaunchKernelGGL(pad_replicate_kernel, frame_grid((long long)(g.h + 32) * (g.w + 32), n), dim3(256), 0, s_i, I[i], Iext[i], n, g.h, g.w);
-        hipLaunchKernelGGL(sobel_kernel, frame_grid((long long)g.h * g.w, n), dim3(256), 0, s_i, I[i], Ixs[i], Iys[i], n, g.h, g.w);
-        hipLaunchKernelGGL(tensor_h_kernel, frame_grid((long long)g.h * g.ws, n), dim3(256), 0, s_i, Ixs[i], Iys[i], aux_i, n, g.h, g.w, g.ws);
-        hipLaunchKernelGGL(tensor_v_kernel, dim3((unsigned)((g.ws + 63) / 64), (unsigned)n, 5u), dim3(64), 0, s_i, aux_i, tensor[i], n, g.h, g.ws, g.hs);
-        VSTAB_HIP(hipGetLastError());
-        if (two_streams && !own) VSTAB_HIP(hipEventRecord(ctx->ev_prep[i], ps));
-    }
-    VSTAB_HIP(hipMemsetAsync(Ul[coarsest], 0, sizeof(float) * (size_t)P * G[coarsest].h * G[coarsest].w, st));
-    VSTAB_HIP(hipMemsetAsync(Vl[coarsest], 0, sizeof(float) * (size_t)P * G[coarsest].h * G[coarsest].w, st));
-
+        if (i == FINEST && i != coarsest) {
+            if (other_pyramid) VSTAB_HIP(hipStreamWaitEvent(D.ps, other_pyramid, 0));
+            if (dis_prep_level(D, i, 0, n, D.ps, D.aux)) return 1;
+            if (two_streams) VSTAB_HIP(hipEventRecord(ctx->ev_prep[i], D.ps));
+            continue;
+        }
+        if (cnt <= 0) continue;
+        if (dis_prep_level(D, i, f0, cnt, own ? st : ps, own ? D.aux_c : (inline_prep ? D.aux_in : D.aux))) return 1;
+        if (two_streams && !own && !inline_prep) VSTAB_HIP(hipEventRecord(ctx->ev_prep[i], ps));
+    }
+    if (pyramid_done) VSTAB_HIP(hipEventRecord(pyramid_done, st));
+    if (other_pyramid) VSTAB_HIP(hipStreamWaitEvent(st, other_pyramid, 0));
+    if (pc > 0) {
+        const size_t o = (size_t)p0 * G[coarsest].h * G[coarsest].w, cnt_px = (size_t)pc * G[coarsest].h * G[coarsest].w;
+        VSTAB_HIP(hipMemsetAsync(D.Ul[coarsest] + o, 0, sizeof(float) * cnt_px, st));
+        VSTAB_HIP(hipMemsetAsync(D.Vl[coarsest] + o, 0, sizeof(float) * cnt_px, st));
+    }
     prep_timer.reset();
-
-    bool grid_fused = false;
-    const float zeta = 0.1f, epsilon = 0.001f, alpha = 20.0f, delta = 5.0f, gamma = 10.0f, omega = 1.6f;
-    const float zeta2 = zeta * zeta, eps2 = epsilon * epsilon, gamma2 = gamma / 2, delta2 = delta / 2, alpha2 = alpha / 4;
-
-    for (int i = coarsest; i >= FINEST; i--) {
-        const LevelGeom& g = G[i];
-        PisArgs pa{};
-        pa.I = I[i]; pa.Iext = Iext[i]; pa.Ix = Ixs[i]; pa.Iy = Iys[i]; pa.tensor = tensor[i];
-        pa.U = Ul[i]; pa.V = Vl[i]; pa.Sx = Sx; pa.Sy = Sy;
-        pa.n = n; pa.w = g.w; pa.h = g.h; pa.ws = g.ws; pa.hs = g.hs;
-        pa.stripe_sz = (int)std::ceil(g.hs / 8.0);
-        pa.spin_limit = 1 << 22;
-#ifdef VSTAB_TEST_HOOKS
-        if (const char* e = getenv("VSTAB_DEBUG_PIS_SPIN_LIMIT")) pa.spin_limit = atoi(e);
-#endif
-        pa.status = ctx->d_status;
-        if (two_streams && i != coarsest) VSTAB_HIP(hipStreamWaitEvent(st, ctx->ev_prep[i], 0));
-        const size_t lds_bytes = (((size_t)(g.w + 32) * (g.h + 32) + 15) & ~size_t(15)) + sizeof(float) * 2 * (size_t)g.hs * g.ws + sizeof(int) * 2 * (size_t)g.hs;
-        VSTAB_REQUIRE(lds_bytes <= 160 * 1024, "vstab_dis_flow_batch: level %dx%d needs %zu B of LDS (> 160 KB)", g.w, g.h, lds_bytes);
-        char kind_pis[24], kind_level[24];
-        snprintf(kind_pis, sizeof(kind_pis), "dis_pis4_L%d", i);
-        snprintf(kind_level, sizeof(kind_level), "dis_level_L%d", i);
-        auto stage_timer = std::make_unique<DetailTimer>(ctx, kind_pis);
-        if (pa.stripe_sz > 4) {
-            if (lds_bytes > 64 * 1024)
-                VSTAB_HIP(hipFuncSetAttribute(reinterpret_cast<const void*>(pis4_kernel<2>), hipFuncAttributeMaxDynamicSharedMemorySize, (int)lds_bytes));
-            hipLaunchKernelGGL(pis4_kernel<2>, dim3((unsigned)P * 2), dim3(64 * 2 * PIS_STRIPES_PER_BLOCK), lds_bytes, st, pa);
-        } else {
-            if (lds_bytes > 64 * 1024)
-                VSTAB_HIP(hipFuncSetAttribute(reinterpret_cast<const void*>(pis4_kernel<1>), hipFuncAttributeMaxDynamicSharedMemorySize, (int)lds_bytes));
-            hipLaunchKernelGGL(pis4_kernel<1>, dim3((unsigned)P * 2), dim3(64 * PIS_STRIPES_PER_BLOCK), lds_bytes, st, pa);
-        }
-        stage_timer.reset();
-        stage_timer = std::make_unique<DetailTimer>(ctx, kind_level);
-        LevelArgs la{};
-#ifdef VSTAB_FUSED_TRACE
-        la.dbg = g_dis_dbg ? g_dis_dbg + 16 * i : nullptr;
-#endif
-        la.I = I[i]; la.Sx = Sx; la.Sy = Sy; la.U = Ul[i]; la.V = Vl[i]; la.vb = vb;
-        la.P = P; la.h = g.h; la.w = g.w; la.ws = g.ws; la.hs = g.hs;
-        la.alpha2 = alpha2; la.delta2 = delta2; la.gamma2 = gamma2; la.zeta2 = zeta2; la.eps2 = eps2; la.omega = omega;
-        if (i > FINEST) {
-            const LevelGeom& d = G[i - 1];
-            la.nextU = Ul[i - 1]; la.nextV = Vl[i - 1]; la.nh = d.h; la.nw = d.w; la.nhs = d.hs; la.nws = d.ws;
-            la.up_sx = 1. / ((double)d.w / g.w); la.up_sy = 1. / ((double)d.h / g.h);
-        }
-        {
-            int tx = 1, ty = 1;
-            auto tile_px = [&](int tx_, int ty_, int& padded) {
-                const int lw = std::min((g.w + tx_ - 1) / tx_ + 2 * SOR_HALO, g.w), lh = std::min((g.h + ty_ - 1) / ty_ + 2 * SOR_HALO, g.h);
-                padded = 2 * ((lw + 3) / 2) * (lh + 2);
-                return ((lw + 1) / 2) * lh;
-            };
-            int padded = 0;
-            while (tile_px(tx, ty, padded) > SOR_NPT * FUSED_T || (size_t)padded * 16 > 160 * 1024) {
-                if ((g.w + tx - 1) / tx >= (g.h + ty - 1) / ty) tx++; else ty++;
-                VSTAB_REQUIRE(tx <= 64 && ty <= 64, "vstab_dis_flow_batch: cannot tile a %dx%d level", g.w, g.h);
-            }
-            la.tiles_x = tx; la.tiles_y = ty; la.lds_plane = (padded + 3) & ~3;
-        }
-        const size_t vr_lds_bytes = sizeof(float) * 4 * (size_t)la.lds_plane;
-        VSTAB_REQUIRE(vr_lds_bytes <= 160 * 1024, "vstab_dis_flow_batch: SOR tile needs %zu B of LDS", vr_lds_bytes);
-        static const int n_cu = [&] { int v = 256; (void)hipDeviceGetAttribute(&v, hipDeviceAttributeMultiprocessorCount, ctx->device); return v; }();
-        bool split = 8 * P < 7 * n_cu;
-        int forced = -1;
-        if (const char* e = getenv("VSTAB_DIS_SPLIT")) { forced = atoi(e); split = forced != 0; }
-        if (split && forced != 2 && la.tiles_x * la.tiles_y == 1) split = false;
-        const bool fuse_grid = !split && i == FINEST && grid_flow != nullptr;
-        if (fuse_grid) {
-            la.grid_out = grid_flow;
-            la.g_h = (h + sample_step - 1) / sample_step; la.g_w = (w + sample_step - 1) / sample_step; la.g_step = sample_step;
-            la.g_sx = 1. / ((double)w / F.w); la.g_sy = 1. / ((double)h / F.h); la.g_mul = (float)(1 << FINEST);
-            grid_fused = true;
-        }
-        if (!split) {
-            if (vr_lds_bytes > 64 * 1024)
-                VSTAB_HIP(hipFuncSetAttribute(reinterpret_cast<const void*>(level_kernel<LEVEL_FUSED>), hipFuncAttributeMaxDynamicSharedMemorySize, (int)vr_lds_bytes));
-            la.parts = 1;
-            hipLaunchKernelGGL(level_kernel<LEVEL_FUSED>, dim3((unsigned)P), dim3(FUSED_T), vr_lds_bytes, st, la);
-        } else {
-            const int px_parts = std::max(1, std::min(64, (g.h * g.w + FUSED_T - 1) / FUSED_T));
-            la.parts = px_parts;
-            hipLaunchKernelGGL(level_kernel<LEVEL_PRE>, dim3((unsigned)(P * px_parts)), dim3(FUSED_T), 0, st, la);
-            hipLaunchKernelGGL(level_kernel<LEVEL_DERIV>, dim3((unsigned)(P * px_parts)), dim3(FUSED_T), 0, st, la);
-            if (vr_lds_bytes > 64 * 1024)
-                VSTAB_HIP(hipFuncSetAttribute(reinterpret_cast<const void*>(level_kernel<LEVEL_TILE>), hipFuncAttributeMaxDynamicSharedMemorySize, (int)vr_lds_bytes));
-            la.parts = la.tiles_x * la.tiles_y;
-            for (int it = 0; it < VAR_ITERS; it++) {
-                la.it = it;
-                hipLaunchKernelGGL(level_kernel<LEVEL_TILE>, dim3((unsigned)(P * la.parts)), dim3(FUSED_T), vr_lds_bytes, st, la);
-            }
-            la.parts = px_parts;
-            hipLaunchKernelGGL(level_kernel<LEVEL_MERGE>, dim3((unsigned)(P * px_parts)), dim3(FUSED_T), 0, st, la);
-            if (la.nextU != nullptr) {
-                la.parts = std::max(1, std::min(64, (la.nhs * la.nws + FUSED_T - 1) / FUSED_T));
-                hipLaunchKernelGGL(level_kernel<LEVEL_UPSAMPLE>, dim3((unsigned)(P * la.parts)), dim3(FUSED_T), 0, st, la);
-            }
-        }
-        VSTAB_HIP(hipGetLastError());
-        stage_timer.reset();
-    }
+    for (int i = coarsest; i > FINEST; i--) {
+        if (two_streams && !inline_prep && i != coarsest) VSTAB_HIP(hipStreamWaitEvent(st, ctx->ev_prep[i], 0));
+        if (int rc = dis_level(ctx, D, i, p0, pc, st, nullptr, 0)) return rc;
+    }
+    return 0;
+}
+
+static int dis_back(vstab_ctx* ctx, DisPlan& D, float* flow, float* grid_flow, int sample_step)
+{
+    hipStream_t st = ctx->stream;
+    const int P = D.P, h = D.h, w = D.w, FINEST = D.FINEST;
+    const LevelGeom& F = D.G[FINEST];
+    if (D.two_streams && FINEST != D.coarsest) VSTAB_HIP(hipStreamWaitEvent(st, ctx->ev_prep[FINEST], 0));
+    if (int rc = dis_level(ctx, D, FINEST, 0, P, st, grid_flow, sample_step)) return rc;
     DetailTimer final_timer(ctx, "dis_final");
     const double fsx = 1. / ((double)w / F.w), fsy = 1. / ((double)h / F.h);
     const float mul = (float)(1 << FINEST);
-    if (grid_flow && !grid_fused) {
+    if (grid_flow && !D.grid_fused) {
         const int gh = (h + sample_step - 1) / sample_step, gw = (w + sample_step - 1) / sample_step;
-        hipLaunchKernelGGL(final_sample_kernel, frame_grid((long long)gh * gw, P), dim3(256), 0, st, Ul[FINEST], Vl[FINEST], grid_flow, P,
+        hipLaunchKernelGGL(final_sample_kernel, frame_grid((long long)gh * gw, P), dim3(256), 0, st, D.Ul[FINEST], D.Vl[FINEST], grid_flow, P,
                            F.h, F.w, gh, gw, sample_step, fsx, fsy, mul);
     }
     if (flow) {
-        hipLaunchKernelGGL(final_sample_kernel, frame_grid((long long)h * w, P), dim3(256), 0, st, Ul[FINEST], Vl[FINEST], flow, P, F.h, F.w,
+        hipLaunchKernelGGL(final_sample_kernel, frame_grid((long long)h * w, P), dim3(256), 0, st, D.Ul[FINEST], D.Vl[FINEST], flow, P, F.h, F.w,
                            h, w, 1, fsx, fsy, mul);
     }
     VSTAB_HIP(hipGetLastError());
     return 0;
+}
+
+static int dis_run(vstab_ctx* ctx, const uint8_t* gray, int n, int h, int w, int FINEST, int coarsest, float* flow, float* grid_flow,
+                   int sample_step)
+{
+    DisPlan D;
+    if (int rc = dis_plan(ctx, n, h, w, FINEST, coarsest, D)) return rc;
+    if (int rc = dis_front(ctx, D, gray, 0, n, 0, n - 1, ctx->stream, false, true, nullptr, nullptr)) return rc;
+    return dis_back(ctx, D, flow, grid_flow, sample_step);
+}
+
+struct DisScales { int f0, c0, f1, c1; bool stateful; };
+static int dis_select_scales(vstab_ctx* ctx, const char* who, int h, int w, DisScales& s)
+{
+    s.f0 = DEFAULT_FINEST; s.c0 = 0;
+    VSTAB_REQUIRE(dis_scales(h, w, s.f0, s.c0), "%s: %dx%d is too small for DIS (OpenCV needs width or height >= 12)", who, w, h);
+    s.f1 = s.f0; s.c1 = 0;
+    VSTAB_REQUIRE(dis_scales(h, w, s.f1, s.c1), "%s: scale selection failed for %dx%d", who, w, h);
+    s.stateful = ctx->dis_first_pair_is_clip_start && (s.c1 != s.c0 || s.f1 != s.f0);
+    return 0;
+}
+
+static int dis_run_clip(vstab_ctx* ctx, const DisScales& s, const uint8_t* gray, int n, int h, int w, float* flow, float* grid_flow,
+                        int sample_step)
+{
+    KernelTimer timer(ctx, "dis");
+    if (!s.stateful) return dis_run(ctx, gray, n, h, w, ctx->dis_first_pair_is_clip_start ? s.f0 : s.f1, ctx->dis_first_pair_is_clip_start ? s.c0 : s.c1, flow, grid_flow, sample_step);
+    if (int rc = dis_run(ctx, gray, 2, h, w, s.f0, s.c0, flow, grid_flow, sample_step)) return rc;
+    if (n == 2) return 0;
+    const int gh = (h + sample_step - 1) / sample_step, gw = (w + sample_step - 1) / sample_step;
+    return dis_run(ctx, gray + (size_t)h * w, n - 1, h, w, s.f1, s.c1, flow ? flow + (size_t)h * w * 2 : nullptr,
+                   grid_flow ? grid_flow + (size_t)gh * gw * 2 : nullptr, sample_step);
 }
 
 extern "C" int vstab_dis_flow_batch(vstab_ctx* ctx, const uint8_t* gray, int n, int h, int w, float* flow, float* grid_flow,
@@ -1599,19 +1715,109 @@
     VSTAB_REQUIRE(flow != nullptr || grid_flow != nullptr, "vstab_dis_flow_batch: no output requested");
     VSTAB_REQUIRE(sample_step >= 1, "vstab_dis_flow_batch: sample_step must be >= 1");
     VSTAB_REQUIRE(h > 0 && w > 0, "vstab_dis_flow_batch: non-positive size");
-    int f0 = DEFAULT_FINEST, c0 = 0;
-    VSTAB_REQUIRE(dis_scales(h, w, f0, c0), "vstab_dis_flow_batch: %dx%d is too small for DIS (OpenCV needs width or height >= 12)", w, h);
-    int f1 = f0, c1 = 0;
-    VSTAB_REQUIRE(dis_scales(h, w, f1, c1), "vstab_dis_flow_batch: scale selection failed for %dx%d", w, h);
+    DisScales s;
+    if (int rc = dis_select_scales(ctx, "vstab_dis_flow_batch", h, w, s)) return rc;
     VSTAB_HIP(hipSetDevice(ctx->device));
+    return dis_run_clip(ctx, s, gray, n, h, w, flow, grid_flow, sample_step);
+}
+
+namespace {
+std::mutex g_front_mutex;
+std::map<vstab_ctx*, FrontEvents> g_front_events;
+
+int front_events(vstab_ctx* ctx, FrontEvents& out)
+{
+    std::lock_guard<std::mutex> lock(g_front_mutex);
+    FrontEvents& fe = g_front_events[ctx];
+    if (!fe.entry) VSTAB_HIP(hipEventCreateWithFlags(&fe.entry, hipEventDisableTiming));
+    if (!fe.grayA) VSTAB_HIP(hipEventCreateWithFlags(&fe.grayA, hipEventDisableTiming));
+    if (!fe.frontA) VSTAB_HIP(hipEventCreateWithFlags(&fe.frontA, hipEventDisableTiming));
+    if (!fe.pyramidA) VSTAB_HIP(hipEventCreateWithFlags(&fe.pyramidA, hipEventDisableTiming));
+    out = fe;
+    return 0;
+}
+}
+
+void vstab_front_release(vstab_ctx* ctx)
+{
+    std::lock_guard<std::mutex> lock(g_front_mutex);
+    auto it = g_front_events.find(ctx);
+    if (it == g_front_events.end()) return;
+    for (hipEvent_t ev : {it->second.entry, it->second.grayA, it->second.frontA, it->second.pyramidA})
+        if (ev) (void)hipEventDestroy(ev);
+    g_front_events.erase(it);
+}
+
+static int front_split(vstab_ctx* ctx, const GrayPlan& gp, DisPlan& D, const FrontEvents& fe, const float* frames, int n, int f1,
+                       uint8_t* gray, float* frame_max, float* grid_flow, int sample_step)
+{
+    hipStream_t st = ctx->stream, side = ctx->side_stream;
+    VSTAB_HIP(hipEventRecord(fe.entry, st));
+    VSTAB_HIP(hipStreamWaitEvent(side, fe.entry, 0));
+    {
+        KernelTimer timer(ctx, "gray");
+        if (int rc = vstab_gray_launch(ctx, gp, frames, 0, f1, gray)) return rc;
+        VSTAB_HIP(hipEventRecord(fe.grayA, st));
+        VSTAB_HIP(hipStreamWaitEvent(side, fe.grayA, 0));
+        if (int rc = dis_front(ctx, D, gray, 0, f1, 0, f1 - 1, side, true, false, nullptr, fe.pyramidA)) return rc;
+        VSTAB_HIP(hipEventRecord(fe.frontA, side));
+        if (int rc = vstab_gray_launch(ctx, gp, frames, f1, n - f1, gray)) return rc;
+        if (frame_max)
+            if (int rc = vstab_gray_range_finish(ctx, gp, n, frame_max)) return rc;
+    }
     KernelTimer timer(ctx, "dis");
-    const bool stateful = ctx->dis_first_pair_is_clip_start && (c1 != c0 || f1 != f0);
-    if (!stateful) return dis_run(ctx, gray, n, h, w, ctx->dis_first_pair_is_clip_start ? f0 : f1, ctx->dis_first_pair_is_clip_start ? c0 : c1, flow, grid_flow, sample_step);
-    if (int rc = dis_run(ctx, gray, 2, h, w, f0, c0, flow, grid_flow, sample_step)) return rc;
-    if (n == 2) return 0;
-    const int gh = (h + sample_step - 1) / sample_step, gw = (w + sample_step - 1) / sample_step;
-    return dis_run(ctx, gray + (size_t)h * w, n - 1, h, w, f1, c1, flow ? flow + (size_t)h * w * 2 : nullptr,
-                   grid_flow ? grid_flow + (size_t)gh * gw * 2 : nullptr, sample_step);
+    if (int rc = dis_front(ctx, D, gray, f1, n, f1 - 1, n - 1, st, false, true, fe.pyramidA, nullptr)) return rc;
+    VSTAB_HIP(hipStreamWaitEvent(st, fe.frontA, 0));
+    return dis_back(ctx, D, nullptr, grid_flow, sample_step);
+}
+
+extern "C" int vstab_gray_dis_batch(vstab_ctx* ctx, const float* frames, int n, int src_h, int src_w, int work_h, int work_w,
+                                    uint8_t* gray, float* frame_max, float* grid_flow, int sample_step, int boundary)
+{
+    if (int rc = vstab_gray_check("vstab_gray_dis_batch", ctx, frames, n, src_h, src_w, work_h, work_w, gray)) return rc;
+    VSTAB_REQUIRE(n >= 2, "vstab_gray_dis_batch: need at least 2 frames, got %d", n);
+    VSTAB_REQUIRE(grid_flow != nullptr, "vstab_gray_dis_batch: grid_flow is NULL");
+    VSTAB_REQUIRE(sample_step >= 1, "vstab_gray_dis_batch: sample_step must be >= 1");
+    VSTAB_REQUIRE(boundary < n, "vstab_gray_dis_batch: boundary %d is not inside the %d frames", boundary, n);
+    DisScales s;
+    if (int rc = dis_select_scales(ctx, "vstab_gray_dis_batch", work_h, work_w, s)) return rc;
+    VSTAB_HIP(hipSetDevice(ctx->device));
+    static const int split_env = [] { const char* e = getenv("VSTAB_FRONT_SPLIT"); return e ? (atoi(e) != 0 ? 1 : 0) : -1; }();
+    const bool split_on = split_env != 0;
+    const int FINEST = ctx->dis_first_pair_is_clip_start ? s.f0 : s.f1, coarsest = ctx->dis_first_pair_is_clip_start ? s.c0 : s.c1;
+    int f1 = 0;
+    if (split_on && boundary != 0 && !s.stateful && !ctx->timing_detail && n >= 3 && coarsest > FINEST) {
+        if (boundary > 0) f1 = boundary;
+        else if (split_env == 1 && dis_fused_form(ctx, n - 1) && getenv("VSTAB_DIS_SPLIT") == nullptr) f1 = n - std::max(1, n / FRONT_TAIL_DIVISOR);
+    }
+    if (f1 <= 0) {
+        {
+            KernelTimer timer(ctx, "gray");
+            GrayPlan gp;
+            if (int rc = vstab_gray_plan(ctx, n, src_h, src_w, work_h, work_w, frame_max != nullptr, &gp)) return rc;
+            if (int rc = vstab_gray_launch(ctx, gp, frames, 0, n, gray)) return rc;
+            if (frame_max)
+                if (int rc = vstab_gray_range_finish(ctx, gp, n, frame_max)) return rc;
+        }
+        return dis_run_clip(ctx, s, gray, n, work_h, work_w, nullptr, grid_flow, sample_step);
+    }
+    FrontEvents fe;
+    if (int rc = front_events(ctx, fe)) return rc;
+    if (!ctx->side_stream) {
+        VSTAB_HIP(hipStreamCreateWithFlags(&ctx->side_stream, hipStreamNonBlocking));
+        VSTAB_HIP(hipEventCreateWithFlags(&ctx->ev_side, hipEventDisableTiming));
+    }
+    GrayPlan gp;
+    if (int rc = vstab_gray_plan(ctx, n, src_h, src_w, work_h, work_w, frame_max != nullptr, &gp)) return rc;
+    DisPlan D;
+    if (int rc = dis_plan(ctx, n, work_h, work_w, FINEST, coarsest, D)) return rc;
+    const int rc = front_split(ctx, gp, D, fe, frames, n, f1, gray, frame_max, grid_flow, sample_step);
+    if (rc != 0) {
+        (void)hipStreamSynchronize(ctx->side_stream);
+        if (ctx->prep_stream) (void)hipStreamSynchronize(ctx->prep_stream);
+        (void)hipStreamSynchronize(ctx->stream);
+    }
+    return rc;
 }
 
 extern "C" int vstab_dis_set_clip_start(vstab_ctx* ctx, int first_pair_is_clip_start)
diff --git a/comfyui-video-stabilizer_amd/csrc/vstab_front.h b/comfyui-video-stabilizer_amd/csrc/vstab_front.h
--- /dev/null
+++ b/comfyui-video-stabilizer_amd/csrc/vstab_front.h
@@ -0,0 +1,23 @@
+#pragma once
+#include "vstab_internal.h"
+
+struct GrayPlan {
+    int src_h = 0, src_w = 0, work_h = 0, work_w = 0;
+    int K = 1, isx = 1, isy = 1;
+    bool same = false, fast = false, fused = false;
+    float* row_max = nullptr;
+    int range_rows = 0;
+    uint8_t* tmp = nullptr;
+    const void *xtab = nullptr, *ytab = nullptr, *xstart = nullptr, *ystart = nullptr;
+};
+
+int vstab_gray_check(const char* who, vstab_ctx* ctx, const float* frames, int n, int src_h, int src_w, int work_h, int work_w,
+                     const uint8_t* gray);
+int vstab_gray_plan(vstab_ctx* ctx, int n, int src_h, int src_w, int work_h, int work_w, bool want_range, GrayPlan* plan);
+int vstab_gray_launch(vstab_ctx* ctx, const GrayPlan& plan, const float* frames, int f0, int count, uint8_t* gray);
+int vstab_gray_range_finish(vstab_ctx* ctx, const GrayPlan& plan, int n, float* frame_max);
+
+struct FrontEvents {
+    hipEvent_t entry = nullptr, grayA = nullptr, frontA = nullptr, pyramidA = nullptr;
+};
+void vstab_front_release(vstab_ctx* ctx);
diff --git a/comfyui-video-stabilizer_amd/csrc/vstab_gray.hip b/comfyui-video-stabilizer_amd/csrc/vstab_gray.hip
--- a/comfyui-video-stabilizer_amd/csrc/vstab_gray.hip
+++ b/comfyui-video-stabilizer_amd/csrc/vstab_gray.hip
@@ -1,4 +1,5 @@
 #include "vstab_internal.h"
+#include "vstab_front.h"
 #include <algorithm>
 #include <cfloat>
 #include <cmath>
@@ -267,15 +268,59 @@
 
 }
 
-static int gray_run(vstab_ctx* ctx, const float* frames, int n, int src_h, int src_w, int work_h, int work_w, uint8_t* gray,
-                    float* frame_max)
-{
-    VSTAB_HIP(hipSetDevice(ctx->device));
+int vstab_gray_plan(vstab_ctx* ctx, int n, int src_h, int src_w, int work_h, int work_w, bool want_range, GrayPlan* plan)
+{
+    GrayPlan& p = *plan;
+    p = GrayPlan{};
+    p.src_h = src_h; p.src_w = src_w; p.work_h = work_h; p.work_w = work_w;
+    const double scale_x = 1. / ((double)work_w / src_w), scale_y = 1. / ((double)work_h / src_h);
+    p.isx = (int)std::lrint(scale_x); p.isy = (int)std::lrint(scale_y);
+    p.same = (work_h == src_h && work_w == src_w);
+    p.fast = !p.same && std::fabs(scale_x - p.isx) < DBL_EPSILON && std::fabs(scale_y - p.isy) < DBL_EPSILON;
+    p.fused = p.fast && p.isx == p.isy && (p.isx == 2 || p.isx == 4);
+    p.K = p.same ? 1 : (p.fused ? p.isx : 1);
+    if (p.fused)
+        VSTAB_REQUIRE(work_w * p.K == src_w && work_h * p.K == src_h, "vstab_gray_downscale: %dx%d is not %d x %dx%d", src_w, src_h, p.K, work_w, work_h);
+    if (want_range) {
+        const int rows = (p.same || !p.fused) ? src_h : work_h;
+        if (ctx->d_range.reserve(sizeof(float) * (size_t)n * rows)) return 1;
+        p.row_max = static_cast<float*>(ctx->d_range.ptr);
+        p.range_rows = rows;
+    }
+    if (!p.same && !p.fused) {
+        if (ctx->d_gray_tmp.reserve((size_t)n * src_h * src_w)) return 1;
+        p.tmp = static_cast<uint8_t*>(ctx->d_gray_tmp.ptr);
+        if (!p.fast) {
+            std::vector<AreaTabEntry> xtab, ytab;
+            std::vector<int> xstart, ystart;
+            build_area_tab(src_w, work_w, scale_x, xtab, xstart);
+            build_area_tab(src_h, work_h, scale_y, ytab, ystart);
+            const size_t b_xt = xtab.size() * sizeof(AreaTabEntry), b_yt = ytab.size() * sizeof(AreaTabEntry);
+            const size_t b_xs = xstart.size() * sizeof(int), b_ys = ystart.size() * sizeof(int);
+            std::vector<unsigned char> blob(b_xt + b_yt + b_xs + b_ys);
+            memcpy(blob.data(), xtab.data(), b_xt);
+            memcpy(blob.data() + b_xt, ytab.data(), b_yt);
+            memcpy(blob.data() + b_xt + b_yt, xstart.data(), b_xs);
+            memcpy(blob.data() + b_xt + b_yt + b_xs, ystart.data(), b_ys);
+            void* d_blob = nullptr;
+            if (vstab_stage_params(ctx, blob.data(), blob.size(), &d_blob)) return 1;
+            const unsigned char* db = static_cast<const unsigned char*>(d_blob);
+            p.xtab = db; p.ytab = db + b_xt; p.xstart = db + b_xt + b_yt; p.ystart = db + b_xt + b_yt + b_xs;
+        }
+    }
+    return 0;
+}
+
+int vstab_gray_launch(vstab_ctx* ctx, const GrayPlan& p, const float* frames, int f0, int count, uint8_t* gray)
+{
+    if (count <= 0) return 0;
     hipStream_t st = ctx->stream;
+    const int src_h = p.src_h, src_w = p.src_w, work_h = p.work_h, work_w = p.work_w;
     const int body = src_w & ~7;
-    KernelTimer timer(ctx, "gray");
-    float* row_max = nullptr;
-    int range_rows = 0;
+    const int n = count;
+    frames += (size_t)f0 * src_h * src_w * 3;
+    gray += (size_t)f0 * work_h * work_w;
+    float* row_max = p.row_max ? p.row_max + (size_t)f0 * p.range_rows : nullptr;
 
     auto threads_for = [](int cols) {
         int best = 256;
@@ -299,80 +344,67 @@
         VSTAB_HIP(hipGetLastError());                                                                                     \
     } while (0)
 
-    const double scale_x = 1. / ((double)work_w / src_w), scale_y = 1. / ((double)work_h / src_h);
-    const int isx = (int)std::lrint(scale_x), isy = (int)std::lrint(scale_y);
-    const bool same = (work_h == src_h && work_w == src_w);
-    const bool fast = !same && std::fabs(scale_x - isx) < DBL_EPSILON && std::fabs(scale_y - isy) < DBL_EPSILON;
-    const bool fused = fast && isx == isy && (isx == 2 || isx == 4);
-    const int K = same ? 1 : (fused ? isx : 1);
-    if (frame_max) {
-        const int rows = (same || !fused) ? src_h : work_h;
-        if (ctx->d_range.reserve(sizeof(float) * (size_t)n * rows)) return 1;
-        row_max = static_cast<float*>(ctx->d_range.ptr);
-        range_rows = rows;
-    }
-    if (same) {
+    if (p.same) {
         LAUNCH_GRAY(1, work_h, gray);
-    } else if (fused) {
-        VSTAB_REQUIRE(work_w * K == src_w && work_h * K == src_h, "vstab_gray_downscale: %dx%d is not %d x %dx%d", src_w, src_h, K, work_w, work_h);
-        if (K == 2) LAUNCH_GRAY(2, work_h, gray);
+    } else if (p.fused) {
+        if (p.K == 2) LAUNCH_GRAY(2, work_h, gray);
         else LAUNCH_GRAY(4, work_h, gray);
     } else {
-        const size_t full = (size_t)n * src_h * src_w;
-        if (ctx->d_gray_tmp.reserve(full)) return 1;
-        uint8_t* tmp = static_cast<uint8_t*>(ctx->d_gray_tmp.ptr);
+        uint8_t* tmp = p.tmp + (size_t)f0 * src_h * src_w;
         LAUNCH_GRAY(1, src_h, tmp);
         const long long out_items = (long long)n * work_h * work_w;
-        if (fast) {
-            hipLaunchKernelGGL(area_int_u8_kernel, dim3(grid_for(out_items)), dim3(256), 0, st, tmp, gray, n, src_h, src_w, work_h, work_w, isx, isy);
-            VSTAB_HIP(hipGetLastError());
+        if (p.fast) {
+            hipLaunchKernelGGL(area_int_u8_kernel, dim3(grid_for(out_items)), dim3(256), 0, st, tmp, gray, n, src_h, src_w, work_h, work_w, p.isx, p.isy);
         } else {
-            std::vector<AreaTabEntry> xtab, ytab;
-            std::vector<int> xstart, ystart;
-            build_area_tab(src_w, work_w, scale_x, xtab, xstart);
-            build_area_tab(src_h, work_h, scale_y, ytab, ystart);
-            const size_t b_xt = xtab.size() * sizeof(AreaTabEntry), b_yt = ytab.size() * sizeof(AreaTabEntry);
-            const size_t b_xs = xstart.size() * sizeof(int), b_ys = ystart.size() * sizeof(int);
-            std::vector<unsigned char> blob(b_xt + b_yt + b_xs + b_ys);
-            memcpy(blob.data(), xtab.data(), b_xt);
-            memcpy(blob.data() + b_xt, ytab.data(), b_yt);
-            memcpy(blob.data() + b_xt + b_yt, xstart.data(), b_xs);
-            memcpy(blob.data() + b_xt + b_yt + b_xs, ystart.data(), b_ys);
-            void* d_blob = nullptr;
-            if (vstab_stage_params(ctx, blob.data(), blob.size(), &d_blob)) return 1;
-            unsigned char* db = static_cast<unsigned char*>(d_blob);
             hipLaunchKernelGGL(area_general_u8_kernel, dim3(grid_for(out_items)), dim3(256), 0, st, tmp, gray, n, src_h, src_w, work_h, work_w,
-                               reinterpret_cast<const AreaTabEntry*>(db), reinterpret_cast<const int*>(db + b_xt + b_yt),
-                               reinterpret_cast<const AreaTabEntry*>(db + b_xt), reinterpret_cast<const int*>(db + b_xt + b_yt + b_xs));
-            VSTAB_HIP(hipGetLastError());
-        }
+                               static_cast<const AreaTabEntry*>(p.xtab), static_cast<const int*>(p.xstart),
+                               static_cast<const AreaTabEntry*>(p.ytab), static_cast<const int*>(p.ystart));
+        }
+        VSTAB_HIP(hipGetLastError());
     }
 #undef LAUNCH_GRAY
-    if (frame_max) {
-        if (ctx->h_peaks_cap < n) {
-            if (ctx->h_peaks) { VSTAB_HIP(hipStreamSynchronize(st)); VSTAB_HIP(hipHostFree(ctx->h_peaks)); ctx->h_peaks = nullptr; ctx->h_peaks_cap = 0; }
-            const int cap = std::max(1024, n);
-            void* hp = nullptr;
-            VSTAB_HIP(hipHostMalloc(&hp, sizeof(float) * (size_t)cap, hipHostMallocMapped | hipHostMallocCoherent));
-            void* dp = nullptr;
-            VSTAB_HIP(hipHostGetDevicePointer(&dp, hp, 0));
-            ctx->h_peaks = static_cast<float*>(hp); ctx->d_peaks_mirror = static_cast<float*>(dp); ctx->h_peaks_cap = cap;
-        }
-        if (!ctx->d_peaks_count) {
-            VSTAB_HIP(hipMalloc(reinterpret_cast<void**>(&ctx->d_peaks_count), 256));
-            VSTAB_HIP(hipMemsetAsync(ctx->d_peaks_count, 0, 256, st));
-        }
-        ctx->peaks_target += (unsigned)n;
-        ctx->peaks_frames = n;
-        hipLaunchKernelGGL(frame_max_kernel, dim3((unsigned)n), dim3(256), 0, st, row_max, frame_max, range_rows, ctx->d_peaks_mirror,
-                           reinterpret_cast<unsigned*>(ctx->d_status) + VSTAB_PEAKS_DONE_WORD, ctx->d_peaks_count, ctx->peaks_target);
-        VSTAB_HIP(hipGetLastError());
-    }
-    return 0;
-}
-
-static int gray_check(const char* who, vstab_ctx* ctx, const float* frames, int n, int src_h, int src_w, int work_h, int work_w,
-                      const uint8_t* gray)
+    return 0;
+}
+
+int vstab_gray_range_finish(vstab_ctx* ctx, const GrayPlan& p, int n, float* frame_max)
+{
+    hipStream_t st = ctx->stream;
+    if (ctx->h_peaks_cap < n) {
+        if (ctx->h_peaks) { VSTAB_HIP(hipStreamSynchronize(st)); VSTAB_HIP(hipHostFree(ctx->h_peaks)); ctx->h_peaks = nullptr; ctx->h_peaks_cap = 0; }
+        const int cap = std::max(1024, n);
+        void* hp = nullptr;
+        VSTAB_HIP(hipHostMalloc(&hp, sizeof(float) * (size_t)cap, hipHostMallocMapped | hipHostMallocCoherent));
+        void* dp = nullptr;
+        VSTAB_HIP(hipHostGetDevicePointer(&dp, hp, 0));
+        ctx->h_peaks = static_cast<float*>(hp); ctx->d_peaks_mirror = static_cast<float*>(dp); ctx->h_peaks_cap = cap;
+    }
+    if (!ctx->d_peaks_count) {
+        VSTAB_HIP(hipMalloc(reinterpret_cast<void**>(&ctx->d_peaks_count), 256));
+        VSTAB_HIP(hipMemsetAsync(ctx->d_peaks_count, 0, 256, st));
+    }
+    const unsigned target = ctx->peaks_target + (unsigned)n;
+    hipLaunchKernelGGL(frame_max_kernel, dim3((unsigned)n), dim3(256), 0, st, p.row_max, frame_max, p.range_rows, ctx->d_peaks_mirror,
+                       reinterpret_cast<unsigned*>(ctx->d_status) + VSTAB_PEAKS_DONE_WORD, ctx->d_peaks_count, target);
+    VSTAB_HIP(hipGetLastError());
+    ctx->peaks_target = target;
+    ctx->peaks_frames = n;
+    return 0;
+}
+
+static int gray_run(vstab_ctx* ctx, const float* frames, int n, int src_h, int src_w, int work_h, int work_w, uint8_t* gray,
+                    float* frame_max)
+{
+    VSTAB_HIP(hipSetDevice(ctx->device));
+    KernelTimer timer(ctx, "gray");
+    GrayPlan plan;
+    if (int rc = vstab_gray_plan(ctx, n, src_h, src_w, work_h, work_w, frame_max != nullptr, &plan)) return rc;
+    if (int rc = vstab_gray_launch(ctx, plan, frames, 0, n, gray)) return rc;
+    if (frame_max) return vstab_gray_range_finish(ctx, plan, n, frame_max);
+    return 0;
+}
+
+int vstab_gray_check(const char* who, vstab_ctx* ctx, const float* frames, int n, int src_h, int src_w, int work_h, int work_w,
+                     const uint8_t* gray)
 {
     VSTAB_REQUIRE(ctx != nullptr, "%s: ctx is NULL", who);
     VSTAB_REQUIRE(frames && gray, "%s: NULL pointer argument", who);
@@ -384,14 +416,14 @@
 extern "C" int vstab_gray_downscale(vstab_ctx* ctx, const float* frames, int n, int src_h, int src_w, int work_h,
                                     int work_w, uint8_t* gray)
 {
-    if (int rc = gray_check("vstab_gray_downscale", ctx, frames, n, src_h, src_w, work_h, work_w, gray)) return rc;
+    if (int rc = vstab_gray_check("vstab_gray_downscale", ctx, frames, n, src_h, src_w, work_h, work_w, gray)) return rc;
     return gray_run(ctx, frames, n, src_h, src_w, work_h, work_w, gray, nullptr);
 }
 
 extern "C" int vstab_gray_downscale_range(vstab_ctx* ctx, const float* frames, int n, int src_h, int src_w, int work_h,
                                           int work_w, uint8_t* gray, float* frame_max)
 {
-    if (int rc = gray_check("vstab_gray_downscale_range", ctx, frames, n, src_h, src_w, work_h, work_w, gray)) return rc;
+    if (int rc = vstab_gray_check("vstab_gray_downscale_range", ctx, frames, n, src_h, src_w, work_h, work_w, gray)) return rc;
     VSTAB_REQUIRE(frame_max != nullptr, "vstab_gray_downscale_range: frame_max is NULL");
     return gray_run(ctx, frames, n, src_h, src_w, work_h, work_w, gray, frame_max);
 }
diff --git a/comfyui-video-stabilizer_amd/distributed.py b/comfyui-video-stabilizer_amd/distributed.py
--- a/comfyui-video-stabilizer_amd/distributed.py
+++ b/comfyui-video-stabilizer_amd/distributed.py
@@ -293,8 +293,7 @@
         if local_frames.shape[0] >= 2:
             def launch(frames):
                 peaks_ = [] if check_value_range else None
-                gray = _fp._gray(ctx, frames, working_size, peaks_)
-                _, grid = ctx.dis_flow_batch(gray, sample_step=_fp.SAMPLE_STEP, want_full=False, want_grid=True, clip_start=(rank == 0))
+                _, grid = _fp._gray_dis(ctx, frames, working_size, peaks_, clip_start=(rank == 0))
                 return ctx.sample_fit_batch_begin(grid, _fp.SAMPLE_STEP, transform_mode), peaks_
 
             pairs_local, peaks = launch(local_frames)
diff --git a/comfyui-video-stabilizer_amd/flow_pipeline.py b/comfyui-video-stabilizer_amd/flow_pipeline.py
--- a/comfyui-video-stabilizer_amd/flow_pipeline.py
+++ b/comfyui-video-stabilizer_amd/flow_pipeline.py
@@ -130,6 +130,14 @@
     if gray_out is not None:
         gray_out.append(gray)
     return gray
+
+
+def _gray_dis(ctx, device_frames, working_size, peaks_out, clip_start=True):
+    if peaks_out is None:
+        return ctx.gray_dis_batch(device_frames, working_size, sample_step=SAMPLE_STEP, clip_start=clip_start)
+    gray, grid, peaks = ctx.gray_dis_batch(device_frames, working_size, sample_step=SAMPLE_STEP, want_range=True, clip_start=clip_start)
+    peaks_out.append(hm.prefetch_peaks(peaks))
+    return gray, grid
 
 
 def estimate_transitions(ctx, device_frames, working_size, transform_mode: str, clip_start: bool = True, peaks_out=None,
@@ -553,8 +561,7 @@
                                 keep_on_device, temporal_fill=0, blocked=None, mask_info=None):
     size = (context.width, context.height)
     peaks = [] if context.range_pending else None
-    gray = _gray(ctx, device_frames, working_size, peaks)
-    _, grid = ctx.dis_flow_batch(gray, sample_step=SAMPLE_STEP, want_full=False, want_grid=True)
+    gray, grid = _gray_dis(ctx, device_frames, working_size, peaks)
     pairs = ctx.sample_fit_batch_begin(grid, SAMPLE_STEP, transform_mode, blocked=blocked)
     ctx.flow_plan_device(ctx.fit_records_device(), pairs, transform_mode, size, working_size, smooth, fps_effective, strength,
                          bool(camera_lock), warp_frames=total_frames, framing=framing_mode)
diff --git a/comfyui-video-stabilizer_amd/native.py b/comfyui-video-stabilizer_amd/native.py
--- a/comfyui-video-stabilizer_amd/native.py
+++ b/comfyui-video-stabilizer_amd/native.py
@@ -152,6 +152,9 @@
     "vstab_dis_flow_batch": (
         C.c_int, [C.c_void_p, C.c_void_p, C.c_int, C.c_int, C.c_int, C.c_void_p, C.c_void_p, C.c_int]),
     "vstab_dis_set_clip_start": (C.c_int, [C.c_void_p, C.c_int]),
+    "vstab_gray_dis_batch": (
+        C.c_int, [C.c_void_p, C.c_void_p, C.c_int, C.c_int, C.c_int, C.c_int, C.c_int, C.c_void_p, C.c_void_p, C.c_void_p, C.c_int,
+                  C.c_int]),
     "vstab_sample_fit_batch": (
         C.c_int, [C.c_void_p, C.c_void_p, C.c_int, C.c_int, C.c_int, C.c_int, C.c_int, C.c_void_p]),
     "vstab_sample_fit_batch_begin": (C.c_int, [C.c_void_p, C.c_void_p, C.c_int, C.c_int, C.c_int, C.c_int, C.c_int]),
@@ -561,6 +564,35 @@
         )
         return flow, grid
 
+    def gray_dis_batch(self, frames, work_size, sample_step=8, want_range=False, clip_start=True, boundary=None):
+        torch = self.torch
+        _check(self.lib.vstab_dis_set_clip_start(self.handle, 1 if clip_start else 0), "vstab_dis_set_clip_start")
+        src = self._as_device_frames(frames)
+        n, sh, sw, ch = src.shape
+        if ch != 3:
+            raise VstabError(f"gray_dis_batch expects 3-channel frames, got {ch}")
+        if n < 2:
+            raise VstabError("gray_dis_batch needs at least two frames")
+        if boundary is None:
+            boundary = min(int(os.environ.get("VSTAB_FRONT_BOUNDARY", "-1")), n - 1)
+        ww, wh = (sw, sh) if work_size is None else (int(work_size[0]), int(work_size[1]))
+        gh, gw = (wh + sample_step - 1) // sample_step, (ww + sample_step - 1) // sample_step
+        gray = torch.empty((n, wh, ww), dtype=torch.uint8, device=self.device)
+        grid = torch.empty((n - 1, gh, gw, 2), dtype=torch.float32, device=self.device)
+        peaks = torch.empty((n,), dtype=torch.float32, device=self.device) if want_range else None
+        self.use_torch_stream()
+        _check(
+            self.lib.vstab_gray_dis_batch(
+                self.handle, _dev_ptr(src), n, sh, sw, wh, ww, _dev_ptr(gray), _dev_ptr(peaks) if peaks is not None else None,
+                _dev_ptr(grid), int(sample_step), int(boundary),
+            ),
+            "vstab_gray_dis_batch",
+        )
+        if want_range:
+            peaks._vstab_fetch = lambda n=n: self.last_frame_peaks(n)
+            return gray, grid, peaks
+        return gray, grid
+
     def tvl1_flow_batch(self, gray, params=None, sample_step=8, want_full=False, want_grid=True, want_iterations=False):
         torch = self.torch
         if gray.device != self.device:
diff --git a/include/vstab.h b/include/vstab.h
--- a/include/vstab.h
+++ b/include/vstab.h
@@ -66,6 +66,9 @@
                          float* flow, float* grid_flow, int sample_step);
 
 int vstab_dis_set_clip_start(vstab_ctx* ctx, int first_pair_is_clip_start);
+
+int vstab_gray_dis_batch(vstab_ctx* ctx, const float* frames, int n, int src_h, int src_w, int work_h, int work_w,
+                         uint8_t* gray, float* frame_max, float* grid_flow, int sample_step, int boundary);
 
 typedef struct vstab_fit_record {
     float matrix[9];
```

New measurement: 29950 frames/s. 7.5% lower.
